# fpusan/moira

Hardware: AMD Instinct MI355X
Metric: reads/sec filtered (300 bp synthetic) (higher is better)
Workload: dtype f64; 1 GPU; BASELINE configs[1]: 10000000 synthetic single-end 300 bp reads, poisson_binomial filter, alpha 0.005, uncert 0.01, resident in HBM (uint8 10000000 x 320, seed 2); reads_per_gpu=10000000, read_length=300, row_stride=320, parallelism=host-side split, 1 rank(s), no data-path collective, world_size=1, mode=bit-exact (no FMA)

## Files before the change

### moira_amd/csrc/mpb_context.cpp

```cpp

#include "mpb_ctx.h"

#include <cstring>
#include <new>


hipError_t Buf::alloc(int64_t bytes)
{
    const hipError_t e = kind == BUF_DEVICE ? hipMalloc(&p, (size_t)bytes)
                                            : hipHostMalloc(&p, (size_t)bytes, kind == BUF_MAPPED ? hipHostMallocMapped : hipHostMallocDefault);
    if (e != hipSuccess) p = nullptr;
    cap = p ? bytes : 0;
    return e;
}

void Buf::release()
{
    if (p) (void)(kind == BUF_DEVICE ? hipFree(p) : hipHostFree(p));
    p = nullptr;
    cap = 0;
}

int Buf::grow(mpb_ctx *c, int64_t bytes, int64_t alloc_bytes)
{
    if (bytes <= cap) return MPB_OK;
    HIPCHK(hipStreamSynchronize(c->stream));
    serve_quiesce(c);
    void *old = p;
    p = nullptr;
    cap = 0;
    if (old) HIPCHK(kind == BUF_DEVICE ? hipFree(old) : hipHostFree(old));
    HIPCHK(alloc(alloc_bytes > bytes ? alloc_bytes : bytes));
    return MPB_OK;
}

int copy_sync(mpb_ctx *c, void *dst, const void *src, size_t bytes, hipMemcpyKind kind)
{
    const hipError_t e_copy = hipMemcpyAsync(dst, src, bytes, kind, c->stream);
    const hipError_t e_sync = hipStreamSynchronize(c->stream);
    HIPCHK_KEPT("hipMemcpyAsync", e_copy);
    HIPCHK_KEPT("hipStreamSynchronize", e_sync);
    return MPB_OK;
}


int mpb_device_count(void)
{
    int n = 0;
    if (hipGetDeviceCount(&n) != hipSuccess) return 0;
    return n;
}

int mpb_create(int device_id, mpb_ctx **out)
{
    if (!out) return fail(MPB_E_INVALID, "mpb_create: out is NULL");
    *out = nullptr;
    int n = mpb_device_count();
    if (n <= 0) return fail(MPB_E_NODEVICE, "no HIP device visible (this library has no CPU path)");
    if (device_id < 0 || device_id >= n)
        return fail(MPB_E_NODEVICE, "device %d out of range (0..%d)", device_id, n - 1);
    HIPCHK(hipSetDevice(device_id));
    mpb_ctx *c = new (std::nothrow) mpb_ctx();
    if (!c) return fail(MPB_E_NOMEM, "host allocation failed");
    c->device = device_id;
    hipError_t e = hipStreamCreateWithFlags(&c->stream, hipStreamNonBlocking);
    if (e == hipSuccess) e = hipStreamCreateWithFlags(&c->copy_stream, hipStreamNonBlocking);
    if (e == hipSuccess) e = hipStreamCreateWithFlags(&c->out_stream, hipStreamNonBlocking);
    for (int k = 0; k < MPB_HOST_SLOTS && e == hipSuccess; k++) {
        e = hipEventCreateWithFlags(&c->slot[k].h2d_done, hipEventDisableTiming);
        if (e == hipSuccess) e = hipEventCreateWithFlags(&c->slot[k].k_done, hipEventDisableTiming);
        if (e == hipSuccess) e = hipEventCreateWithFlags(&c->slot[k].d2h_done, hipEventDisableTiming);
    }
    c->copy_threads = staging_threads();
    auto tables = [c](Carver &k) { k.take(c->d_lut, 256); k.take(c->d_lut_odds, 256); k.take(c->d_lut_private, 256); };
    Carver size;
    tables(size);
    if (e == hipSuccess) e = c->luts.alloc(size.bytes());
    if (e == hipSuccess) {
        Carver place(c->luts.p);
        tables(place);
        MpbPair both[2][256], (&h)[256] = both[0];
        build_lut(both[0], both[1]);
        c->narrow_ok = true;
        for (int qq = 1; qq < 255; qq++) {
            volatile double d = 1.0 - h[qq].y;
            if (memcmp((const void *)&d, &h[qq].x, sizeof(double)) != 0) c->narrow_ok = false;
        }
        e = hipMemcpyAsync(c->d_lut, both, sizeof(both), hipMemcpyHostToDevice, c->stream);
        const hipError_t e_sync = hipStreamSynchronize(c->stream);
        if (e == hipSuccess) e = e_sync;
    }
    if (e == hipSuccess) e = c->pin_mem.alloc(sizeof(PinWords));
    c->pin = (PinWords *)c->pin_mem.p;
    if (e == hipSuccess) {
        hipDeviceProp_t prop;
        e = hipGetDeviceProperties(&prop, device_id);
        if (e == hipSuccess) c->n_cu = prop.multiProcessorCount;
    }
    if (e != hipSuccess) {
        int rc = fail(MPB_E_HIP, "context setup failed: %s", hipGetErrorString(e));
        mpb_destroy(c);
        return rc;
    }
    *out = c;
    return MPB_OK;
}

int mpb_destroy(mpb_ctx *c)
{
    if (!c) return MPB_OK;
    (void)hipSetDevice(c->device);
    serve_free(c);
    if (c->stream) (void)hipStreamSynchronize(c->stream);
    if (c->copy_stream) (void)hipStreamSynchronize(c->copy_stream);
    if (c->out_stream) (void)hipStreamSynchronize(c->out_stream);
    for (auto &sl : c->slot) {
        if (sl.h2d_done) (void)hipEventDestroy(sl.h2d_done);
        if (sl.k_done) (void)hipEventDestroy(sl.k_done);
        if (sl.d2h_done) (void)hipEventDestroy(sl.d2h_done);
    }
    for (auto &s : c->spans) { (void)hipEventDestroy(s.a); (void)hipEventDestroy(s.b); }
    for (auto ev : c->event_pool) (void)hipEventDestroy(ev);
    if (c->stream) (void)hipStreamDestroy(c->stream);
    if (c->copy_stream) (void)hipStreamDestroy(c->copy_stream);
    if (c->out_stream) (void)hipStreamDestroy(c->out_stream);
    delete c;
    return MPB_OK;
}

int mpb_device_lut(mpb_ctx *c, double *a_out, double *b_out)
{
    CTXCHK(c);
    if (!a_out || !b_out) return fail(MPB_E_INVALID, "mpb_device_lut: NULL output");
    double2 h[256];
    int rc = copy_sync(c, h, c->d_lut, sizeof(h), hipMemcpyDeviceToHost);
    if (rc) return rc;
    for (int q = 0; q < 256; q++) { a_out[q] = h[q].x; b_out[q] = h[q].y; }
    return MPB_OK;
}

int mpb_stream(mpb_ctx *c, void **stream_out)
{
    CTXCHK(c);
    if (!stream_out) return fail(MPB_E_INVALID, "stream_out is NULL");
    *stream_out = (void *)c->stream;
    return MPB_OK;
}

int mpb_synchronize(mpb_ctx *c)
{
    CTXCHK(c);
    HIPCHK(hipStreamSynchronize(c->stream));
    return MPB_OK;
}

int mpb_malloc(mpb_ctx *c, int64_t bytes, void **dptr_out)
{
    CTXCHK(c);
    if (!dptr_out || bytes < 0) return fail(MPB_E_INVALID, "mpb_malloc: bad arguments");
    *dptr_out = nullptr;
    HIPCHK(hipMalloc(dptr_out, bytes > 0 ? (size_t)bytes : 16));
    return MPB_OK;
}

int mpb_free(mpb_ctx *c, void *dptr)
{
    CTXCHK(c);
    HIPCHK(hipStreamSynchronize(c->stream));
    serve_quiesce(c);
    if (dptr) HIPCHK(hipFree(dptr));
    return MPB_OK;
}

int mpb_memcpy_h2d(mpb_ctx *c, void *dst, const void *src, int64_t bytes)
{
    CTXCHK(c);
    if (bytes < 0 || (bytes > 0 && (!dst || !src))) return fail(MPB_E_INVALID, "mpb_memcpy_h2d: bad arguments");
    if (bytes == 0) return MPB_OK;
    return copy_sync(c, dst, src, (size_t)bytes, hipMemcpyHostToDevice);
}

int mpb_memcpy_d2h(mpb_ctx *c, void *dst, const void *src, int64_t bytes)
{
    CTXCHK(c);
    if (bytes < 0 || (bytes > 0 && (!dst || !src))) return fail(MPB_E_INVALID, "mpb_memcpy_d2h: bad arguments");
    if (bytes == 0) return MPB_OK;
    return copy_sync(c, dst, src, (size_t)bytes, hipMemcpyDeviceToHost);
}

int mpb_memset(mpb_ctx *c, void *dst, int value, int64_t bytes)
{
    CTXCHK(c);
    if (bytes < 0 || (bytes > 0 && !dst)) return fail(MPB_E_INVALID, "mpb_memset: bad arguments");
    if (bytes == 0) return MPB_OK;
    HIPCHK(hipMemsetAsync(dst, value, (size_t)bytes, c->stream));
    return MPB_OK;
}

int mpb_host_alloc(mpb_ctx *c, int64_t bytes, void **hptr_out)
{
    CTXCHK(c);
    if (!hptr_out || bytes < 0) return fail(MPB_E_INVALID, "mpb_host_alloc: bad arguments");
    *hptr_out = nullptr;
    HIPCHK(hipHostMalloc(hptr_out, bytes > 0 ? (size_t)bytes : 16, hipHostMallocDefault));
    return MPB_OK;
}

int mpb_host_free(mpb_ctx *c, void *hptr)
{
    CTXCHK(c);
    drain_pipeline(c);
    serve_quiesce(c);
    if (hptr) HIPCHK(hipHostFree(hptr));
    return MPB_OK;
}


int ensure_workspace(mpb_ctx *c, int64_t n)
{
    if (!c->ws_small.p) {
        int rc = c->ws_small.grow(c, sizeof(MpbSmallBlock));
        if (rc) return rc;
        HIPCHK(hipMemsetAsync(c->ws_small.p, 0, sizeof(MpbSmallBlock), c->stream));
        MpbSmallBlock *b = (MpbSmallBlock *)c->ws_small.p;
        c->ws.tables = &b->tables;
        c->ws.tables2 = &b->tables2;
        c->ws.ovf_count = &b->ovf_count;
        c->ws.bad_len = &b->bad_len;
        c->ws.pass_count = &b->pass_count;
        c->ws.ovf_total = &b->ovf_total;
        c->ws.wide_count = &b->wide_count;
        c->ws.alg_cells = &b->alg_cells;
        c->ws.nar_count = &b->nar_count;
        c->ws.nar_sample = b->nar_sample;
        c->ws.pt_count = &b->pt_count;
        c->ws.lut = c->d_lut;
    }
    if (n <= c->ws_cap) return MPB_OK;
    c->ws_cap = 0;
    const int64_t cap = n + n / 8 + 1024;
    const int64_t nb = (cap + MPB_PRE_READS - 1) / MPB_PRE_READS;
    MpbWorkspace &w = c->ws;
    int rc = carve(c, c->ws_block, [&w, cap, nb](Carver &k) {
        k.take(w.cls, cap);
        k.take(w.perm, cap + (int64_t)MPB_NCLS * 64);
        k.take(w.perm_ns, cap + (int64_t)MPB_NCLS * 64);
        k.take(w.blockhist, nb * MPB_SKEYS);
        k.take(w.ovf_list, cap);
    });
    if (rc) return rc;
    c->ws_cap = cap;
    return MPB_OK;
}

int ensure_wide_workspace(mpb_ctx *c, int64_t n)
{
    if (n <= c->ws_wide_cap) return MPB_OK;
    c->ws_wide_cap = 0;
    const int64_t cap = n + n / 8 + 1024;
    MpbWorkspace &w = c->ws;
    int rc = carve(c, c->ws_wide, [&w, cap](Carver &k) { k.take(w.wide_list, cap); k.take(w.wide_rows, cap); });
    if (rc) return rc;
    c->ws_wide_cap = cap;
    return MPB_OK;
}

int ensure_narrow_workspace(mpb_ctx *c, int64_t n, bool ragged)
{
    const int64_t cap = n + n / 8 + 1024;
    MpbWorkspace &w = c->ws;
    int rc;
    if (n > c->ws_nar_cap) {
        c->ws_nar_cap = 0;
        rc = carve(c, c->ws_nar, [&w, cap](Carver &k) {
            k.take(w.nar_seg, cap + 64);
            k.take(w.nar_list, cap + 64);
            k.take(w.nar_wave_count, MPB_NAR_MAX_WAVES + 1);
        });
        if (rc) return rc;
        c->ws_nar_cap = cap;
    }
    if (ragged && n > c->ws_rg_cap) {
        c->ws_rg_cap = 0;
        rc = carve(c, c->ws_rg, [&w, cap](Carver &k) {
            k.take(w.rg_ord, cap + 64);
            k.take(w.rg_gpre, cap / 64 + 2);
            k.take(w.rg_wsum, cap / 4096 + 2);
            k.take(w.rg_wpre, cap / 4096 + 2);
            k.take(w.rg_gstart, MPB_NAR_MAX_WAVES + 1);
        });
        if (rc) return rc;
        c->ws_rg_cap = cap;
        if (!c->rg_per_cu[0]) mpb_narrow_rg_blocks_per_cu(c->rg_per_cu);
    }
    return MPB_OK;
}

int PrivateTable::install(const double2 *h)
{
    int rc = ensure_workspace(c, 1);
    if (rc) return rc;
    if ((rc = copy_sync(c, c->d_lut_private, h, 256 * sizeof(double2), hipMemcpyHostToDevice))) return rc;
    c->ws.lut = c->d_lut_private;
    on = true;
    return MPB_OK;
}


static hipEvent_t get_event(mpb_ctx *c)
{
    if (!c->event_pool.empty()) { hipEvent_t e = c->event_pool.back(); c->event_pool.pop_back(); return e; }
    hipEvent_t e = nullptr;
    (void)hipEventCreate(&e);
    return e;
}


void Span::start()
{
    a = get_event(c); b = get_event(c);
    (void)hipEventRecord(a, c->stream);
}

static int resolve_spans(mpb_ctx *c)
{
    if (c->spans.empty()) return MPB_OK;
    HIPCHK(hipStreamSynchronize(c->stream));
    for (auto &s : c->spans) {
        float ms = 0.f;
        if (hipEventElapsedTime(&ms, s.a, s.b) == hipSuccess) { c->acc_ms[s.kid] += ms; c->acc_n[s.kid] += 1; }
        c->event_pool.push_back(s.a);
        c->event_pool.push_back(s.b);
    }
    c->spans.clear();
    return MPB_OK;
}

int mpb_timing_enable(mpb_ctx *c, int on) { CTXCHK(c); c->timing = on != 0; return MPB_OK; }

int mpb_timing_reset(mpb_ctx *c)
{
    CTXCHK(c);
    int rc = resolve_spans(c);
    if (rc) return rc;
    for (int k = 0; k < MPB_K_COUNT; k++) { c->acc_ms[k] = 0; c->acc_n[k] = 0; }
    return MPB_OK;
}

int mpb_kernel_time(mpb_ctx *c, int kid, double *total_ms, int64_t *launches)
{
    CTXCHK(c);
    if (kid < 0 || kid >= MPB_K_COUNT) return fail(MPB_E_INVALID, "kernel id %d out of range", kid);
    int rc = resolve_spans(c);
    if (rc) return rc;
    if (total_ms) *total_ms = c->acc_ms[kid];
    if (launches) *launches = c->acc_n[kid];
    return MPB_OK;
}
```

### moira_amd/csrc/mpb_ctx.h

```cpp
#ifndef MPB_CTX_H
#define MPB_CTX_H

#include "../../include/moira_pb.h"
#include "mpb_internal.h"
#include "mpb_host_internal.h"
#include "mpb_hostonly.h"

#include <vector>

static_assert(sizeof(MpbPair) == sizeof(double2) && offsetof(MpbPair, y) == sizeof(double), "MpbPair is double2's layout");

static inline int hip_fail(const char *what, hipError_t e)
{
    return fail(e == hipErrorOutOfMemory ? MPB_E_NOMEM : MPB_E_HIP, "%s failed: %s", what, hipGetErrorString(e));
}
#define HIPCHK(expr)                                        \
    do {                                                    \
        hipError_t e_ = (expr);                             \
        if (e_ != hipSuccess) return hip_fail(#expr, e_);   \
    } while (0)
#define HIPCHK_KEPT(what, e)                                \
    do {                                                    \
        if ((e) != hipSuccess) return hip_fail(what, e);    \
    } while (0)

#define CTXCHK(c)                                                     \
    do {                                                              \
        if (!(c)) return fail(MPB_E_INVALID, "%s: ctx is NULL", __func__); \
        HIPCHK(hipSetDevice((c)->device));                            \
    } while (0)

enum BufKind { BUF_DEVICE, BUF_PINNED, BUF_MAPPED };
struct Buf {
    BufKind kind;
    void *p = nullptr;
    int64_t cap = 0;
    explicit Buf(BufKind k = BUF_DEVICE) : kind(k) {}
    Buf(const Buf &) = delete;
    Buf &operator=(const Buf &) = delete;
    ~Buf() { release(); }
    hipError_t alloc(int64_t bytes);
    int grow(mpb_ctx *c, int64_t bytes, int64_t alloc_bytes = 0);
    void release();
};

struct Carver {
    char *base;
    int64_t off = 0;
    explicit Carver(void *b = nullptr) : base((char *)b) {}
    template <typename T> void take(T *&ptr, int64_t count)
    {
        ptr = base ? (T *)(base + off) : nullptr;
        off += align_up(count * (int64_t)sizeof(T), 256);
    }
    int64_t bytes() const { return off; }
};
template <typename Layout>
static int carve(mpb_ctx *c, Buf &b, Layout &&layout, int headroom = 1)
{
    Carver size;
    layout(size);
    int rc = b.grow(c, size.bytes(), size.bytes() * headroom);
    if (rc) return rc;
    Carver place(b.p);
    layout(place);
    return MPB_OK;
}

struct MpbSmallBlock {
    alignas(256) MpbTables tables;
    alignas(256) MpbTables tables2;
    alignas(64) int32_t ovf_count;
    alignas(64) int32_t bad_len;
    alignas(64) unsigned long long pass_count;
    alignas(64) long long ovf_total;
    alignas(64) int32_t wide_count;
    alignas(64) unsigned long long alg_cells;
    alignas(64) int32_t nar_count;
    alignas(64) int32_t nar_sample[MPB_NAR_BUCKETS + 2];
    alignas(64) int32_t pt_count;
};

struct PinWords {
    int32_t nar_count;
    int32_t n_overflow;
    unsigned long long n_pass;
    int32_t bad_len;
    int32_t bad255;
    int32_t sample[MPB_NAR_BUCKETS + 2];
    int32_t pt_handed;
    unsigned long long pt_kept;
    long long ovf_total;
    int64_t text_status[2];
    uint32_t fq_head[4];
    int64_t fq_status[4];
    uint32_t fq_head2[4];
    int64_t fq_status2[4];
    int64_t pair_status[4];
    uint32_t pair_head[MPB_PAIR_HEAD_WORDS];
    int64_t fmt_words[2];
};

struct TimedSpan { int kid; hipEvent_t a, b; };

struct ChunkArrays {
    uint8_t *q; int32_t *len; double *ee; int32_t *ns; uint8_t *pass;
    void in(Carver &k, int64_t m, int64_t row_stride) { k.take(q, m * row_stride); k.take(len, m); }
    void out(Carver &k, int64_t m) { k.take(ee, m); k.take(ns, m); k.take(pass, m); }
};

#define MPB_HOST_SLOTS 4
struct HostSlot {
    Buf dev{BUF_DEVICE}, pin_in{BUF_PINNED}, pin_out{BUF_PINNED};
    ChunkArrays d{}, hin{}, hout{};
    hipEvent_t h2d_done = nullptr, k_done = nullptr, d2h_done = nullptr;
    int64_t off = -1, m = 0;
};

struct mpb_ctx {
    int device = -1;
    hipStream_t stream = nullptr;
    hipStream_t copy_stream = nullptr;
    hipStream_t out_stream = nullptr;
    HostSlot slot[MPB_HOST_SLOTS];
    int copy_threads = 1;
    Buf luts{BUF_DEVICE};
    double2 *d_lut = nullptr;
    double2 *d_lut_odds = nullptr;
    double2 *d_lut_private = nullptr;
    MpbWorkspace ws{};
    Buf ws_small{BUF_DEVICE};
    Buf ws_block{BUF_DEVICE};
    int64_t ws_cap = 0;
    struct Classified {
        bool valid = false; const uint8_t *q = nullptr; int64_t n = 0, stride = 0; const int32_t *len = nullptr;
        int32_t fixed_len = 0; mpb_filter_params params{}; double *ee = nullptr; int32_t *ns = nullptr; uint8_t *pass = nullptr;
    } classified;
    Buf ws_wide{BUF_DEVICE};
    int64_t ws_wide_cap = 0;
    bool timing = false;
    std::vector<TimedSpan> spans;
    std::vector<hipEvent_t> event_pool;
    double acc_ms[MPB_K_COUNT] = {0};
    int64_t acc_n[MPB_K_COUNT] = {0};
    Buf stage{BUF_DEVICE};
    Buf pin_host{BUF_MAPPED};
    uint32_t small_token = 0;
    int n_cu = 0;
    bool narrow_ok = false;
    Buf ws_nar{BUF_DEVICE};
    int64_t ws_nar_cap = 0;
    Buf ws_rg{BUF_DEVICE}; int64_t ws_rg_cap = 0;
    Buf pt_rec{BUF_DEVICE};
    int rg_per_cu[MPB_NRG_FORMS] = {0};
    Buf text_stage{BUF_DEVICE};
    Buf contig_stage{BUF_DEVICE};
    Buf contig_tabs{BUF_DEVICE};
    bool contig_tabs_ready = false;
    Buf bgzf_stage{BUF_DEVICE};
    Buf inflate_stage{BUF_DEVICE};
    Buf fastq_stage{BUF_DEVICE};
    Buf fastq_index{BUF_DEVICE};
    Buf format_stage{BUF_DEVICE};
    Buf format_out{BUF_DEVICE};
    struct ResidentText {
        int64_t gen = 0, last = 0;
        const uint8_t *text = nullptr; int64_t text_bytes = 0; const int64_t *idx = nullptr; int64_t n = 0;
    } resident;
    Buf pin_mem{BUF_PINNED};
    PinWords *pin = nullptr;
    struct NarrowChoice {
        bool valid = false; int64_t n = 0, stride = 0; int32_t fixed_len = 0; double alpha = 0; uint32_t flags = 0;
        int rows0 = 0; int split = 0; int calls = 0;
        double expect_back = 0;
    } nar_choice;
    mpb_path_info last_path{};
    bool classes_whole = true;
    struct CtxServe {
        bool tried = false, ok = false, running = false;
        hipStream_t stream = nullptr;
        Buf pin{BUF_MAPPED}, dev{BUF_DEVICE};
        MpbServeBox box{};
        uint32_t generation = 0, tok = 0;
        double cached_alpha = -1.0;
        MpbDevParams cached_prm;
    } serve;
};

struct Span {
    mpb_ctx *c; int kid; hipEvent_t a = nullptr, b = nullptr;
    Span(mpb_ctx *c_, int kid_) : c(c_), kid(kid_) { if (c->timing) start(); }
    void start();
    ~Span()
    {
        if (c->timing) { (void)hipEventRecord(b, c->stream); c->spans.push_back({kid, a, b}); }
    }
};

#include "mpb_queue.h"

struct PrivateTable {
    mpb_ctx *c;
    bool on = false;
    explicit PrivateTable(mpb_ctx *ctx) : c(ctx) {}
    int install(const double2 *h);
    ~PrivateTable() { if (on) c->ws.lut = c->d_lut; }
};

int copy_sync(mpb_ctx *c, void *dst, const void *src, size_t bytes, hipMemcpyKind kind);
int ensure_workspace(mpb_ctx *c, int64_t n);
int ensure_wide_workspace(mpb_ctx *c, int64_t n);
int ensure_narrow_workspace(mpb_ctx *c, int64_t n, bool ragged);
MpbDevParams make_dev_params(const mpb_filter_params *p, int32_t fixed_len, int32_t max_len);
void drain_pipeline(mpb_ctx *c);
int filter_host_pipeline(mpb_ctx *c, const uint8_t *q, int64_t n, int64_t row_stride, const int32_t *len, int32_t fixed_len,
                         const mpb_filter_params *params, double *ee, int32_t *ns, uint8_t *pass, mpb_filter_counts *counts,
                         int poisson);
struct TextStage {
    uint8_t *text; mpb_text_row *rows; int64_t *status; uint8_t *q; int32_t *len; uint8_t *flags;
    double *ee; int32_t *ns; uint8_t *pass;
    void layout(Carver &k, int64_t text_bytes, int64_t n, int64_t piece_rows, int64_t stride)
    {
        k.take(text, align_up(text_bytes > 0 ? text_bytes : 1, 16));
        k.take(rows, n);
        layout_results(k, n, piece_rows, stride);
    }
    void layout_results(Carver &k, int64_t n, int64_t piece_rows, int64_t stride)
    {
        k.take(status, 2);
        k.take(q, piece_rows * stride);
        k.take(len, n); k.take(flags, n);
        k.take(ee, n); k.take(ns, n); k.take(pass, n);
    }
};
int64_t text_piece_rows(int64_t n, int64_t stride);
int filter_text_pieces(StreamQueue &q, const uint8_t *d_text, int64_t text_bytes, const mpb_text_row *d_rows, int64_t n, int64_t stride,
                       int64_t piece_rows, int32_t fastq_offset, int32_t lower_n_is_base, const mpb_filter_params *params,
                       int32_t poisson, const TextStage &st, int64_t *n_pass, int64_t *n_overflow, int64_t *bad_record);
struct TextResults {
    double *ee; int32_t *ns; uint8_t *pass; int32_t *len; uint8_t *flags;
    std::vector<int32_t> len_tmp;
    int32_t *len_host() const { return len ? len : len_tmp.empty() ? nullptr : const_cast<int32_t *>(len_tmp.data()); }
};
static inline bool text_host_tail(const mpb_filter_params *params, int32_t poisson)
{
    return poisson && !(params && (params->flags & MPB_FLAG_POISSON_DEVICE_TAIL));
}
int text_results_queue(StreamQueue &q, const TextStage &st, int64_t n, bool host_tail, TextResults &r);
int text_results_tail(int64_t n, const mpb_filter_params *params, bool host_tail, const TextResults &r, int64_t *n_pass);
int text_results_out(StreamQueue &q, const TextStage &st, int64_t n, const mpb_filter_params *params, int32_t poisson, TextResults &r,
                     int64_t *n_pass);

struct FastqStage {
    uint8_t *text; uint32_t *info, *prefix, *head; int64_t *status;
    void layout(Carver &k, int64_t text_bytes, int64_t n_tiles)
    {
        k.take(text, align_up(text_bytes > 0 ? text_bytes : 1, 16));
        k.take(info, n_tiles > 0 ? n_tiles : 1);
        k.take(prefix, n_tiles > 0 ? n_tiles : 1);
        k.take(head, 4);
        k.take(status, 4);
    }
};

struct FastqIndex {
    uint32_t *start; int64_t *idx; uint8_t *kinds; mpb_text_row *desc;
    void layout(Carver &k, int64_t n_start, int64_t rows)
    {
        k.take(start, n_start);
        k.take(idx, rows * MPB_IDX_COLS);
        k.take(kinds, rows);
        k.take(desc, rows);
    }
};

struct Indexed {
    FastqStage st{};
    FastqIndex ix{};
    int64_t n = 0, rows = 0, longest = 0;
};
void fastq_index_queue_head(StreamQueue &q, Indexed &out, int64_t text_bytes, int32_t final, uint32_t *pin_head = nullptr);
int fastq_index_finish(StreamQueue &q, int64_t text_bytes, int64_t max_records, int32_t max_len, int64_t idx_cap_rows, int64_t *n_needed,
                       Indexed &out, int32_t *why);
void queue_index_out(StreamQueue &q, const Indexed &in, int64_t *idx_out, uint32_t *consumed32, uint8_t *kind8);
struct FastqFilterAsk {
    int32_t fastq_offset, lower_n_is_base; const mpb_filter_params *params; int32_t poisson;
    mpb_filter_counts *counts; int64_t *bad_record;
};
int filter_indexed(StreamQueue &q, const Indexed &in, int64_t text_bytes, uint8_t *text_out, int64_t *idx_out, int64_t *n,
                   int64_t *consumed, int32_t *bad_kind, const FastqFilterAsk &ask, TextResults &r);
void resident_keep(mpb_ctx *c, const Indexed &in, int64_t text_bytes);
void resident_drop(mpb_ctx *c);
struct BgzfStage {
    uint8_t *text; uint32_t *tok; uint8_t *slots; uint32_t *size, *mstat, *crc; int64_t *off; uint8_t *out;
    void layout(Carver &k, int64_t members)
    {
        k.take(text, align_up(members * (int64_t)MPB_BGZF_DATA, 16));
        k.take(tok, members * (int64_t)MPB_BGZF_DATA);
        k.take(slots, members * (int64_t)MPB_BGZF_SLOT);
        k.take(size, members); k.take(mstat, members * 4); k.take(crc, members);
        k.take(off, members + 1);
        k.take(out, members * ((int64_t)MPB_BGZF_DATA + 31));
    }
};
struct BgzfHost {
    std::vector<uint32_t> crc, mstat;
    std::vector<int64_t> off;
    int reserve(int64_t per_piece);
};
int64_t bgzf_piece_members(int64_t members);
int bgzf_compress_piece(StreamQueue &q, const BgzfStage &st, int64_t tb, int64_t nm, const uint8_t *host_text,
                        const mpb_crc_range *d_ranges, uint32_t *d_bad, BgzfHost &h, uint8_t *out, int64_t out_room, int64_t *got_out,
                        mpb_bgzf_stats *stats);
void serve_quiesce(mpb_ctx *c);
void serve_free(mpb_ctx *c);

#endif
```

### moira_amd/csrc/mpb_internal.h

```cpp
#ifndef MPB_INTERNAL_H
#define MPB_INTERNAL_H

#include <hip/hip_runtime.h>
#include "mpb_shared.h"

#define MPB_TILE_MAX_ROWS 1024
#define MPB_WIDE_WAVES 16
#define MPB_MAX_ROWS (MPB_TILE_MAX_ROWS * MPB_WIDE_WAVES)
#define MPB_MAX_STRIDE 65536
#define MPB_SMALL_MAX_STRIDE 16384

struct MpbClass { int cap, G, R; };

#define MPB_NCLS 32
#define MPB_CLASSES(X)                                                                       \
    X(0, 2, 1) X(1, 3, 1) X(2, 4, 1) X(3, 5, 1) X(4, 6, 1) X(5, 7, 1) X(6, 8, 1) X(7, 9, 1)  \
    X(8, 10, 1) X(9, 12, 1) X(10, 14, 1) X(11, 16, 1)                                        \
    X(12, 10, 2) X(13, 12, 2) X(14, 14, 2) X(15, 16, 2)                                      \
    X(16, 10, 4) X(17, 12, 4) X(18, 14, 4) X(19, 16, 4)                                      \
    X(20, 9, 8) X(21, 10, 8) X(22, 11, 8) X(23, 12, 8) X(24, 14, 8) X(25, 16, 8)             \
    X(26, 10, 16) X(27, 12, 16) X(28, 16, 16)                                                \
    X(29, 12, 32) X(30, 16, 32) X(31, 16, 64)

#define MPB_THIN_CLASSES(X)                                                                  \
    X(0, 1, 2) X(1, 1, 4) X(2, 1, 8) X(3, 1, 16) X(4, 1, 32) X(5, 1, 64) X(6, 2, 64)         \
    X(7, 4, 64) X(8, 8, 64) X(9, 16, 64)

#define MPB_CLASS_ENTRY(ID, RR, GG) {(RR) * (GG), GG, RR},
#define MPB_CLASS_TABLE { MPB_CLASSES(MPB_CLASS_ENTRY) }

#define MPB_PRE_ROUNDS 4
#define MPB_PRE_READS (256 * MPB_PRE_ROUNDS)
#define MPB_CLS_SETTLED 0x7f
#define MPB_CLS_WIDE 0x7e

#define MPB_LEN_SHIFT 6
#define MPB_LEN_BINS (1024 >> MPB_LEN_SHIFT)
#define MPB_SKEYS (MPB_NCLS * MPB_LEN_BINS)

struct MpbTables {
    int32_t count[MPB_NCLS];
    int32_t perm_base[MPB_NCLS + 1];
    int32_t tile_start[MPB_NCLS + 1];
    int32_t total_tiles;
    int32_t kcount[MPB_SKEYS];
    int32_t key_base[MPB_SKEYS];
};

#define MPB_DP_CHUNK 8

struct MpbDevParams {
    double thr;
    double uncert;
    double maxerrors;
    float  z;
    float  zq;
    float  clow;
    int32_t ambig_mode;
    uint32_t flags;
    int32_t fixed_len;
    int32_t max_len;
    int32_t len_shift;
};

struct MpbWorkspace {
    uint8_t  *cls;
    int32_t  *perm;
    uint16_t *perm_ns;
    int32_t  *blockhist;
    MpbTables *tables;
    MpbTables *tables2;
    int32_t  *ovf_list;
    int32_t  *ovf_count;
    int32_t  *bad_len;
    long long *ovf_total;
    int32_t  *wide_list;
    int32_t  *wide_rows;
    int32_t  *wide_count;
    unsigned long long *pass_count;
    unsigned long long *alg_cells;
    const double2 *lut;
    int32_t  *nar_count;
    int32_t  *nar_seg;
    int32_t  *nar_list;
    int32_t  *nar_wave_count;
    int32_t  *nar_sample;
    int2     *rg_ord;
    int32_t  *rg_gpre;
    unsigned long long *rg_wsum, *rg_wpre;
    int32_t  *rg_gstart;
    int32_t  *pt_count;
};

#define MPB_NAR_MAX_WAVES 8192
#define MPB_NAR_AUTO_MIN_READS (1 << 18)

#define MPB_LUT_BYTES   (256 * 16)
#define MPB_LAMBDA_MAX_STRIDE (1 << 24)

void mpb_launch_prepass(const uint8_t *q, int64_t n, int64_t stride, const int32_t *len,
                        const MpbDevParams &prm, const MpbWorkspace &ws, int32_t *ns_out,
                        double *ee_out, uint8_t *pass_out, hipStream_t s, const int32_t *list = nullptr);
void mpb_launch_decode_classify(const uint8_t *seq, const uint8_t *qual, int32_t offset, uint8_t *out, int32_t *err,
                                int64_t n, int64_t stride, const int32_t *len, const MpbDevParams &prm,
                                const MpbWorkspace &ws, int32_t *ns_out, double *ee_out, uint8_t *pass_out, hipStream_t s);
void mpb_launch_encode(const uint8_t *q, int64_t n, int64_t stride, int32_t offset, uint8_t *seq, uint8_t *qual, hipStream_t s);
struct MpbSmallHost {
    uint8_t *stage;
    int32_t *ns_dev;
    uint32_t *done;
    uint32_t token;
};
void mpb_launch_small(const uint8_t *q, int64_t n, int64_t stride, const int32_t *len, const MpbDevParams &prm,
                      const MpbWorkspace &ws, int32_t *ns, double *ee, uint8_t *pass, hipStream_t s,
                      const MpbSmallHost *host = nullptr);
#define MPB_SERVE_STRIDE 2048
struct alignas(64) MpbServePrm { MpbDevParams p; };
struct MpbServeBox {
    const uint8_t *q;
    int64_t stride;
    const MpbServePrm *prm;
    const unsigned long long *door;
    uint32_t *done;
    double *ee; int32_t *ns; uint8_t *pass;
    int64_t q_step, prm_step, door_step, done_step, ee_step, ns_step, pass_step;
    const uint32_t *stop;
    uint32_t *exited;
    uint8_t *stage;
    int32_t *ns_dev; uint8_t *cls; int32_t *ident;
    uint32_t *gone;
    int32_t n_ent;
};
void mpb_launch_serve(const MpbServeBox &box, const double2 *lut, uint32_t generation, uint32_t lifetime_ms, hipStream_t s);
void mpb_launch_scan(int64_t n, const int32_t *len, const MpbWorkspace &ws, hipStream_t s);
void mpb_launch_scatter(int64_t n, const int32_t *len, const int32_t *ns, const MpbDevParams &prm, const MpbWorkspace &ws,
                        hipStream_t s, const int32_t *list = nullptr);
void mpb_launch_dp(const uint8_t *q, int64_t n, int64_t stride, const int32_t *len,
                   const MpbDevParams &prm, const MpbWorkspace &ws, const int32_t *ns,
                   double *ee, uint8_t *pass, hipStream_t s, const double2 *lut_odds = nullptr);
void mpb_launch_overflow(const uint8_t *q, int64_t n, int64_t stride, const int32_t *len,
                         const MpbDevParams &prm, const MpbWorkspace &ws, const int32_t *ns,
                         double *ee, uint8_t *pass, hipStream_t s);
void mpb_launch_wide(const uint8_t *q, int64_t stride, const int32_t *len, const MpbDevParams &prm,
                     const MpbWorkspace &ws, const int32_t *ns, double *ee, uint8_t *pass, hipStream_t s);
void mpb_launch_lambda(const uint8_t *q, int64_t n, int64_t stride, const int32_t *len, int32_t fixed_len,
                       const double2 *lut_ap, double *lambda, int32_t *ns, int32_t *bad, hipStream_t s);
#define MPB_PT_LAMBDA_MAX 64.0
#define MPB_PT_WINDOW 0x1p-17
struct MpbPoissonRec { double lambda; int32_t idx, ns, len, pad_; };
struct MpbPoissonFix { double ee; int32_t idx, pass; };
void mpb_launch_poisson_tail(const double *lambda, const int32_t *ns, const int32_t *len, int64_t n, const MpbDevParams &prm,
                             double *ee, uint8_t *pass, int32_t *handed, MpbPoissonRec *rec, int32_t rec_cap,
                             unsigned long long *n_pass, hipStream_t s);
void mpb_launch_poisson_patch(const MpbPoissonFix *fix, int32_t m, double *ee, uint8_t *pass, hipStream_t s);
void mpb_launch_decode(const uint8_t *seq, const uint8_t *qual, int64_t n, int64_t stride, const int32_t *len,
                       int32_t fixed_len, int32_t offset, uint8_t *out, int32_t *err, hipStream_t s);
void mpb_launch_count(const uint8_t *pass, int64_t n, const MpbWorkspace &ws, hipStream_t s);
void mpb_launch_pack_text(const uint8_t *text, int64_t text_bytes, const mpb_text_row *rows, int64_t n, int64_t k0, int32_t offset,
                          bool lower_n_is_base, int64_t stride, uint8_t *out, int32_t *len_out, uint8_t *flags_out,
                          int64_t *status, hipStream_t s);
#define MPB_RG_MAX_STRIDE 4096
#define MPB_NRG_FORMS 8
#define MPB_NRG_EXACT_FORMS 5
#define MPB_NAR_GRID_CAP_MAX 2048
void mpb_launch_narrow(int rows0, int split_chunks, const uint8_t *q, int64_t n, int64_t stride, int32_t fixed_len, const int32_t *len,
                       const MpbDevParams &prm, const MpbWorkspace &ws, double *ee, int32_t *ns, uint8_t *pass, int n_cu,
                       const int *rg_per_cu, int grid_cap, int *waves, hipStream_t s, const double2 *lut_odds = nullptr);
void mpb_narrow_rg_blocks_per_cu(int per_cu[MPB_NRG_FORMS]);
void mpb_launch_sample(const uint8_t *q, int64_t n, int64_t stride, int32_t fixed_len, const int32_t *len, const MpbDevParams &prm,
                       const MpbWorkspace &ws, int n_sample, hipStream_t s);
struct MpbContigArgs;
void mpb_launch_contigs(const MpbContigArgs &a, hipStream_t s);
void mpb_launch_contig_rows(const int64_t *out_idx, const uint8_t *done, int64_t n, int64_t rec_cap, int32_t max_len, int64_t stride,
                            mpb_text_row *rows, hipStream_t s);
#define MPB_BGZF_SLOT 65536
void mpb_launch_bgzf_deflate(const uint8_t *text, int64_t text_bytes, int64_t n_members, uint32_t *tok, uint8_t *slots,
                             uint32_t *size, uint32_t *mstat, hipStream_t s);
void mpb_launch_bgzf_scan(const uint32_t *size, int64_t n_members, int64_t *off, hipStream_t s);
void mpb_launch_bgzf_frame(const uint8_t *slots, const uint32_t *size, const int64_t *off, const uint32_t *crc, int64_t text_bytes,
                           int64_t n_members, int64_t out_cap, uint8_t *out, hipStream_t s);
#define MPB_INFLATE_MSTAT 8
void mpb_launch_bgzf_inflate(const uint8_t *in, int64_t in_bytes, const mpb_bgzf_member_row *rows, int64_t n_members, uint8_t *text,
                             int64_t text_bytes, uint32_t *mstat, hipStream_t s);
#define MPB_FQ_TILE 16384
void mpb_launch_fq_lines(const uint8_t *text, int64_t text_bytes, int64_t n_tiles, uint32_t *info, hipStream_t s);
void mpb_launch_fq_scan(const uint8_t *text, int64_t text_bytes, bool final_text, const uint32_t *info, int64_t n_tiles,
                        uint32_t *prefix, uint32_t *head, hipStream_t s);
void mpb_launch_fq_starts(const uint8_t *text, int64_t text_bytes, int64_t n_tiles, const uint32_t *prefix, const uint32_t *head,
                          uint32_t *start, int64_t n_start, hipStream_t s);
void mpb_launch_fq_rows(const uint8_t *text, int64_t text_bytes, const uint32_t *start, int64_t n_start, int64_t n, int32_t max_len,
                        int64_t *idx, uint8_t *kinds, mpb_text_row *desc, int64_t *status, hipStream_t s);
#define MPB_CRC_RANGE_MAX 65536
struct mpb_crc_range { int64_t off; int32_t len, pad; };
void mpb_launch_bgzf_crc32(const uint8_t *text, int64_t text_bytes, const mpb_crc_range *ranges, int64_t n, uint32_t *crc,
                           uint32_t *bad, hipStream_t s);
#define MPB_PAIR_HEAD_WORDS 32
struct MpbLdsClasses;
void mpb_launch_pair_rows(const int64_t *fidx, const int64_t *ridx, int64_t m, const uint8_t *ftext, int64_t fbytes, const uint8_t *rtext,
                          int64_t rbytes, int maxabs, bool take, const MpbLdsClasses &classes, mpb_pair_row *rows, int8_t *cls,
                          int64_t *status, hipStream_t s);
void mpb_launch_pair_count(const mpb_pair_row *rows, const int8_t *cls, int64_t n, uint32_t *table, uint32_t *prefix, uint32_t *head,
                           int64_t *status, hipStream_t s);
void mpb_launch_pair_lists(const int8_t *cls, int64_t n, const uint32_t *prefix, const uint32_t *head, int32_t *list, hipStream_t s);
struct FmParams;
void mpb_launch_fmt_count(const uint8_t *text, const int64_t *idx, const int64_t *sel, const int64_t *relabel_index,
                          const int32_t *label_id, int64_t nsel, const FmParams &p, int64_t *size, int64_t *prefix, int64_t *head,
                          int64_t *status, hipStream_t s);
void mpb_launch_fmt_write(const uint8_t *text, const uint8_t *blob, const int64_t *idx, const int64_t *sel,
                          const int64_t *relabel_index, const int32_t *label_id, int64_t k0, int64_t k1, const FmParams &p,
                          const int64_t *prefix, const int64_t *status, int64_t win_lo, int64_t win_hi, uint8_t *out, hipStream_t s);
void mpb_launch_synth(uint8_t *q, int64_t n, int64_t stride, int32_t fixed_len, int32_t min_len,
                      int32_t max_len, int32_t *len, uint64_t seed, int64_t first_read,
                      hipStream_t s, int32_t profile = 0);

#endif
```

### moira_amd/csrc/mpb_kernels.hip

```cpp

#include "mpb_internal.h"
#include <cstdlib>
#include <cstdio>
#include "../../include/mpb_synth.h"

#pragma clang fp contract(off)

__shared__ double2 mpb_s_lut[256];
__shared__ unsigned long long mpb_s_cells;

namespace {

__constant__ MpbClass c_classes[MPB_NCLS] = MPB_CLASS_TABLE;

struct ClassOfRows {
    uint8_t t[MPB_TILE_MAX_ROWS + 1];
    constexpr ClassOfRows() : t{}
    {
        constexpr MpbClass cl[MPB_NCLS] = MPB_CLASS_TABLE;
        for (int rows = 0; rows < MPB_TILE_MAX_ROWS + 1; rows++) {
            int c = 0;
            for (int k = 0; k < MPB_NCLS - 1; k++) c += (rows > cl[k].cap) ? 1 : 0;
            t[rows] = (uint8_t)c;
        }
    }
};
__constant__ ClassOfRows c_class_of_rows{};

__device__ __forceinline__ int lane_id() { return threadIdx.x & 63; }

template <typename T>
__device__ __forceinline__ T gload(const T *p)
{
    return *(const __attribute__((address_space(1))) T *)(p);
}
typedef uint32_t u32x4 __attribute__((ext_vector_type(4)));
__device__ __forceinline__ uint4 gload16(const uint8_t *p)
{
    const u32x4 x = *(const __attribute__((address_space(1))) u32x4 *)(p);
    return make_uint4(x.x, x.y, x.z, x.w);
}
template <typename T>
__device__ __forceinline__ void gstore(T *p, T v)
{
    *(__attribute__((address_space(1))) T *)(p) = v;
}

__device__ __forceinline__ void wave_lds_fence()
{
    __builtin_amdgcn_fence(__ATOMIC_RELEASE, "wavefront");
    __builtin_amdgcn_s_waitcnt(0xc07f);
    __builtin_amdgcn_wave_barrier();
    __builtin_amdgcn_fence(__ATOMIC_ACQUIRE, "wavefront");
}

__device__ __forceinline__ int clamp_len(int li, int max_len) { return min(max(li, 0), max_len); }

__device__ __forceinline__ bool settled_by_chernoff(const MpbDevParams &prm, float mu, int li)
{
    if (!(prm.flags & MPB_FLAG_DECISION_ONLY)) return false;
    const float t = mu * (1.0f - 1e-4f) - prm.clow * sqrtf(mu) - 0.02f;
    return mu > 1.0f && (double)floorf(t) > mpb_limit(prm, li);
}

typedef float f32x2 __attribute__((ext_vector_type(2)));

__device__ __forceinline__ uint32_t mask_dword(uint32_t w, int nvalid_bytes)
{
    if (nvalid_bytes >= 4) return w;
    if (nvalid_bytes <= 0) return 0u;
    return w & ((1u << (8 * nvalid_bytes)) - 1u);
}

__device__ __forceinline__ uint32_t fill_dword(uint32_t w, int nvalid_bytes)
{
    if (nvalid_bytes >= 4) return w;
    if (nvalid_bytes <= 0) return 0xFEFEFEFEu;
    const uint32_t m = (1u << (8 * nvalid_bytes)) - 1u;
    return (w & m) | (0xFEFEFEFEu & ~m);
}

#define MPB_PRE_NB 5
#define MPB_MARK_UPPER 128.0f
#define MPB_MARK_LOWER 65536.0f

__device__ __forceinline__ void pre_chunk(const float2 *tab, const uint4 x, f32x2 &a01, float &s3)
{
    const uint32_t ww[4] = {x.x, x.y, x.z, x.w};
#pragma unroll
    for (int d = 0; d < 4; d++)
#pragma unroll
        for (int t = 0; t < 4; t++) {
            const float2 e = tab[(ww[d] >> (8 * t)) & 0xffu];
            a01 += (f32x2){e.x, e.y};
            s3 = __builtin_fmaf(e.x, e.y, s3);
        }
}

__device__ __forceinline__ uint32_t decode4_bytes(uint32_t sw, uint32_t qw, int nv, int offset, int &bad)
{
    uint32_t ow = 0;
#pragma unroll
    for (int t = 0; t < 4; t++) {
        const uint32_t b = (sw >> (8 * t)) & 0xffu;
        int qv = (int)((qw >> (8 * t)) & 0xffu) - offset;
        uint32_t o = 0;
        if (t < nv) {
            if (qv < 0) { bad++; qv = 1; }
            if (qv > 254) { bad++; qv = 254; }
            if (qv == 0) qv = 1;
            o = b == 'N' ? 0u : b == 'n' ? 255u : (uint32_t)qv;
        }
        ow |= o << (8 * t);
    }
    return ow;
}

__device__ __forceinline__ uint32_t zero_bytes(uint32_t x)
{
    return ~(((x & 0x7f7f7f7fu) + 0x7f7f7f7fu) | x) & 0x80808080u;
}

__device__ __forceinline__ uint32_t decode4(uint32_t sw, uint32_t qw, int nv, int offset, uint32_t off4, int &bad)
{
    const uint32_t H = 0x80808080u;
    const uint32_t d = ((qw | H) - (off4 & ~H)) ^ ((qw ^ ~off4) & H);
    uint32_t lt = ((~qw & off4) | (~(qw ^ off4) & d)) & H;
    uint32_t keep = 0xffffffffu;
    if (nv < 4) keep = nv <= 0 ? 0u : ((1u << (8 * nv)) - 1u);
    lt &= keep;
    if (lt) return decode4_bytes(sw, qw, nv, offset, bad);
    uint32_t q = d + (zero_bytes(d) >> 7);
    const uint32_t amb = zero_bytes((sw | 0x20202020u) ^ 0x6e6e6e6eu);
    const uint32_t amb_full = (amb << 1) - (amb >> 7);
    const uint32_t lower_full = ((sw >> 5) & 0x01010101u) * 255u;
    q = (amb_full & lower_full) | (~amb_full & q);
    return q & keep;
}

__device__ __forceinline__ uint4 decode16(const uint4 sq, const uint4 ql, int pos0, int li, int offset, int &bad)
{
    const int nv = li - pos0;
    if (offset < 1)
        return make_uint4(decode4_bytes(sq.x, ql.x, nv, offset, bad), decode4_bytes(sq.y, ql.y, nv - 4, offset, bad),
                          decode4_bytes(sq.z, ql.z, nv - 8, offset, bad), decode4_bytes(sq.w, ql.w, nv - 12, offset, bad));
    const uint32_t off4 = (uint32_t)(offset & 0xff) * 0x01010101u;
    if (offset > 255) {
        return make_uint4(decode4_bytes(sq.x, ql.x, nv, offset, bad), decode4_bytes(sq.y, ql.y, nv - 4, offset, bad),
                          decode4_bytes(sq.z, ql.z, nv - 8, offset, bad), decode4_bytes(sq.w, ql.w, nv - 12, offset, bad));
    }
    return make_uint4(decode4(sq.x, ql.x, nv, offset, off4, bad), decode4(sq.y, ql.y, nv - 4, offset, off4, bad),
                      decode4(sq.z, ql.z, nv - 8, offset, off4, bad), decode4(sq.w, ql.w, nv - 12, offset, off4, bad));
}

__device__ __forceinline__ uint32_t lower_as_q254(uint32_t w)
{
    return w ^ (zero_bytes(~w) >> 7);
}

__device__ __forceinline__ void pre_dword_again(const float2 *tab, uint32_t w, f32x2 &a01, float &s3)
{
    w = lower_as_q254(w);
#pragma unroll 1
    for (int t = 0; t < 4; t++) {
        const float2 e = tab[(w >> (8 * t)) & 0xffu];
        a01 += (f32x2){e.x, e.y};
        s3 = __builtin_fmaf(e.x, e.y, s3);
    }
}

struct PreDecode {
    const uint8_t *seq;
    const uint8_t *qual;
    uint8_t *out;
    int32_t offset;
    int32_t *err;
};

struct PreOut {
    uint8_t *cls; int32_t *ns; double *ee; uint8_t *pass;
    int32_t *bad_len, *wide_list, *wide_rows, *wide_count;
};

__device__ __forceinline__ void class_read(int64_t i, float mu, float var, float k3, uint32_t ambi, int li, bool bad, bool ragged,
                                           const MpbDevParams &prm, const PreOut &o, int *s_hist, int nb)
{
    const int nzero = (int)(ambi & 0xffffu), n255 = (int)(ambi >> 16);
    const float v = fmaxf(var, 1e-12f);
    const float x = mu + prm.z * sqrtf(v) + (k3 / v) * prm.zq;
    int rows = (int)floorf(fminf(x, 1e9f) + 0.5f) + 1;
    if (prm.flags & MPB_FLAG_TEST_UNDERPREDICT) rows = rows / 2;
    const int scored = li - nzero - n255;
    rows = min(rows, scored + 1);
    rows = max(rows, 1);
    o.ns[i] = bad ? 0 : nzero + n255;
    const int c = c_class_of_rows.t[min(rows, MPB_TILE_MAX_ROWS)];
    const bool settled = !bad && settled_by_chernoff(prm, mu, li);
    const bool empty = !bad && scored <= 0 && !(1.0 > prm.thr);
    if (bad) {
        atomicAdd(o.bad_len, 1);
        o.cls[i] = (uint8_t)MPB_CLS_SETTLED;
        o.ee[i] = __builtin_nan("");
        o.pass[i] = 0;
    } else if (empty) {
        double e = mpb_add_ns(prm, 0.0, nzero + n255);
        const bool keep = mpb_round_and_keep(prm, e, nzero > 0, li);
        o.cls[i] = (uint8_t)(MPB_CLS_SETTLED | (nzero > 0 ? 0x80 : 0));
        o.ee[i] = e;
        o.pass[i] = (uint8_t)(keep ? 1 : 0);
    } else if (settled) {
        o.cls[i] = (uint8_t)(MPB_CLS_SETTLED | (nzero > 0 ? 0x80 : 0));
        o.ee[i] = __builtin_inf();
        o.pass[i] = 0;
    } else if (rows > MPB_TILE_MAX_ROWS) {
        const int pos = atomicAdd(o.wide_count, 1);
        o.wide_list[pos] = (int32_t)i;
        o.wide_rows[pos] = rows;
        o.cls[i] = (uint8_t)(MPB_CLS_WIDE | (nzero > 0 ? 0x80 : 0));
    } else {
        o.cls[i] = (uint8_t)(c | (nzero > 0 ? 0x80 : 0));
        atomicAdd(&s_hist[c * nb + (ragged ? min(MPB_LEN_BINS - 1, li >> prm.len_shift) : 0)], 1);
    }
}

template <bool RAGGED, bool LONG, bool LISTED>
__global__ __launch_bounds__(256) void k_prepass(const uint8_t *__restrict__ q, int64_t n,
                                                 int64_t stride, const int32_t *__restrict__ len_arg,
                                                 MpbDevParams prm, PreOut o, int32_t *__restrict__ blockhist,
                                                 const int32_t *__restrict__ list)
{
    __shared__ float2 s_tab[256];
    __shared__ float4 s_row[4][64];
    __shared__ int s_hist[RAGGED ? MPB_SKEYS : MPB_NCLS];
    const int32_t *__restrict__ len = RAGGED ? len_arg : nullptr;
    constexpr int nb = RAGGED ? MPB_LEN_BINS : 1;
    const int tid = threadIdx.x, w = tid >> 6, lane = tid & 63;
    {
        const bool amb = tid == 0 || tid == 255;
        float p = __builtin_amdgcn_exp2f(-0.33219281f * (float)tid);
        p = amb ? 0.0f : p;
        s_tab[tid] = make_float2(p, tid == 0 ? MPB_MARK_UPPER : tid == 255 ? MPB_MARK_LOWER : p * (1.0f - p));
    }
    for (int k = tid; k < MPB_NCLS * nb; k += 256) s_hist[k] = 0;
    __syncthreads();

    const int r16 = lane & 15, cl = lane >> 4;
    for (int round = 0; round < MPB_PRE_ROUNDS; round++) {
    const int64_t wave_row0 = (int64_t)blockIdx.x * MPB_PRE_READS + round * 256 + w * 64;
    if (wave_row0 >= n) break;

    for (int rb = 0; rb < 64; rb += 16) {
        const bool live = wave_row0 + rb + r16 < n;
        const int64_t i = LISTED ? (live ? (int64_t)list[wave_row0 + rb + r16] : 0) : wave_row0 + rb + r16;
        const int li = live ? (len ? clamp_len(len[i], prm.max_len) : prm.fixed_len) : 0;
        int ncol = (li + 15) >> 4;
        int nfull = live ? (li >> 4) : (1 << 20);
        if (len || wave_row0 + 64 > n) {
#pragma unroll
            for (int off = 8; off >= 1; off >>= 1) {
                ncol = max(ncol, __shfl_xor(ncol, off));
                nfull = min(nfull, __shfl_xor(nfull, off));
            }
        }
        ncol = __builtin_amdgcn_readfirstlane(ncol);
        nfull = __builtin_amdgcn_readfirstlane(nfull);
        const uint8_t *src = q + (live ? i : (int64_t)0) * stride + cl * 16;
        float mu = 0.f, var = 0.f, k3 = 0.f;
        uint32_t ambi = 0;
        auto panel = [&](const int pb, const int pend) {
        f32x2 a01 = {0.f, 0.f};
        float s3 = 0.f;
        for (int cb = pb; cb < pend; cb += 4 * MPB_PRE_NB) {
            uint4 xs[MPB_PRE_NB];
#pragma unroll
            for (int b = 0; b < MPB_PRE_NB; b++) {
                const int c0 = cb + 4 * b;
                xs[b] = make_uint4(0, 0, 0, 0);
                if (c0 < pend && li > (c0 + cl) * 16)
                    xs[b] = *reinterpret_cast<const uint4 *>(src + c0 * 16);
            }
#pragma unroll
            for (int b = 0; b < MPB_PRE_NB; b++) {
                const int c0 = cb + 4 * b;
                if (c0 >= pend) break;
                uint4 y = xs[b];
                if (c0 + 4 > nfull) {
                    const int nv = li - (c0 + cl) * 16;
                    y.x = fill_dword(y.x, nv); y.y = fill_dword(y.y, nv - 4);
                    y.z = fill_dword(y.z, nv - 8); y.w = fill_dword(y.w, nv - 12);
                }
                pre_chunk(s_tab, y, a01, s3);
            }
        }
        const float n255 = floorf(a01.y * (1.0f / MPB_MARK_LOWER));
        if (n255 > 0.0f) {
            a01 = (f32x2){0.f, 0.f};
            s3 = 0.f;
#pragma unroll 1
            for (int c0 = pb; c0 < pend; c0 += 4) {
                const int nv = li - (c0 + cl) * 16;
                if (nv <= 0) break;
#pragma unroll 1
                for (int d = 0; d < 4; d++)
                    pre_dword_again(s_tab, fill_dword(*reinterpret_cast<const uint32_t *>(src + c0 * 16 + d * 4), nv - 4 * d), a01, s3);
            }
        }
        const float rem = a01.y;
        const float nzero = floorf(rem * (1.0f / MPB_MARK_UPPER));
        const float pvar = rem - MPB_MARK_UPPER * nzero;
        mu += a01.x;
        var += pvar;
        k3 += pvar - 2.0f * s3;
        ambi += (uint32_t)nzero + ((uint32_t)n255 << 16);
        };
        if (LONG) { for (int pb = 0; pb < ncol; pb += 12 * MPB_PRE_NB) panel(pb, min(ncol, pb + 12 * MPB_PRE_NB)); }
        else panel(0, ncol);
#pragma unroll
        for (int off = 16; off <= 32; off <<= 1) {
            mu += __shfl_xor(mu, off);
            var += __shfl_xor(var, off);
            k3 += __shfl_xor(k3, off);
            ambi += __shfl_xor(ambi, off);
        }
        const float amb = __uint_as_float(ambi);
        if (cl == 0) s_row[w][rb + r16] = make_float4(mu, var, k3, amb);
    }
    wave_lds_fence();
    {
        const int64_t k = wave_row0 + lane;
        if (k < n) {
            const int64_t i = LISTED ? (int64_t)list[k] : k;
            const float4 e = s_row[w][lane];
            const int li = len ? clamp_len(len[i], prm.max_len) : prm.fixed_len;
            class_read(i, e.x, e.y, e.z, __float_as_uint(e.w), li, RAGGED && li != len[i], RAGGED, prm, o, s_hist, nb);
        }
    }
    wave_lds_fence();
    }
    __syncthreads();
    for (int k = tid; k < MPB_NCLS * nb; k += 256) blockhist[(int64_t)k * gridDim.x + blockIdx.x] = s_hist[k];
}

#define MPB_LIN_K 5
#define MPB_LIN_CHUNKS (256 * MPB_LIN_K)

template <bool RAGGED, bool DECODE>
__global__ __launch_bounds__(256) void k_classify_linear(const uint8_t *__restrict__ q, int64_t n, int64_t stride,
                                                         const int32_t *__restrict__ len_arg, MpbDevParams prm, PreOut o,
                                                         int32_t *__restrict__ blockhist, PreDecode dec, uint32_t cpr_magic)
{
    __shared__ float2 s_tab[256];
    __shared__ float4 s_part[MPB_LIN_CHUNKS];
    __shared__ int s_len[MPB_PRE_READS];
    __shared__ int s_hist[RAGGED ? MPB_SKEYS : MPB_NCLS];
    const int32_t *__restrict__ len = RAGGED ? len_arg : nullptr;
    constexpr int nb = RAGGED ? MPB_LEN_BINS : 1;
    const int tid = threadIdx.x;
    {
        const bool amb = tid == 0 || tid == 255;
        float p = __builtin_amdgcn_exp2f(-0.33219281f * (float)tid);
        p = amb ? 0.0f : p;
        s_tab[tid] = make_float2(p, tid == 0 ? MPB_MARK_UPPER : tid == 255 ? MPB_MARK_LOWER : p * (1.0f - p));
    }
    for (int k = tid; k < MPB_NCLS * nb; k += 256) s_hist[k] = 0;
    const int cpr = (int)(stride >> 4);
    const int tile_rows = max(1, min(MPB_PRE_READS, MPB_LIN_CHUNKS / cpr));
    const int64_t first = (int64_t)blockIdx.x * MPB_PRE_READS;
    const int64_t last = min(n, first + MPB_PRE_READS);
    int lpr = 1;
    while (lpr < 64 && lpr * 2 * tile_rows <= 256) lpr *= 2;
    int badq = 0;
    for (int64_t row0 = first; row0 < last; row0 += tile_rows) {
        const int nr = (int)min((int64_t)tile_rows, last - row0);
        const int nchunks = nr * cpr;
        __syncthreads();
        for (int t = tid; t < nr; t += 256) s_len[t] = len ? clamp_len(len[row0 + t], prm.max_len) : prm.fixed_len;
        __syncthreads();
        const int64_t base = row0 * stride;
        uint4 xs[MPB_LIN_K], ys[MPB_LIN_K];
        int nvs[MPB_LIN_K];
#pragma unroll
        for (int k = 0; k < MPB_LIN_K; k++) {
            const int c = tid + k * 256;
            xs[k] = ys[k] = make_uint4(0, 0, 0, 0);
            nvs[k] = -1;
            if (c < nchunks) {
                const int r = cpr_magic ? (int)__umulhi((uint32_t)c, cpr_magic) : c;
                const int col = c - r * cpr;
                const int nv = s_len[r] - col * 16;
                nvs[k] = max(nv, 0);
                if (nv > 0) {
                    if (DECODE) {
                        xs[k] = *reinterpret_cast<const uint4 *>(dec.seq + base + (int64_t)c * 16);
                        ys[k] = *reinterpret_cast<const uint4 *>(dec.qual + base + (int64_t)c * 16);
                    } else {
                        xs[k] = *reinterpret_cast<const uint4 *>(q + base + (int64_t)c * 16);
                    }
                }
            }
        }
        __builtin_amdgcn_sched_barrier(0);
#pragma unroll
        for (int k = 0; k < MPB_LIN_K; k++) {
            const int c = tid + k * 256;
            const int nv = nvs[k];
            if (nv < 0) continue;
            uint4 y = xs[k];
            if (DECODE) {
                if (nv > 0) y = decode16(xs[k], ys[k], 0, nv, dec.offset, badq);
                *reinterpret_cast<uint4 *>(dec.out + base + (int64_t)c * 16) = y;
            }
            float4 part = make_float4(0.f, 0.f, 0.f, __int_as_float(0));
            if (nv > 0) {
                if (nv < 16) {
                    y.x = fill_dword(y.x, nv); y.y = fill_dword(y.y, nv - 4);
                    y.z = fill_dword(y.z, nv - 8); y.w = fill_dword(y.w, nv - 12);
                }
                f32x2 a01 = {0.f, 0.f};
                float s3 = 0.f;
                pre_chunk(s_tab, y, a01, s3);
                const float n255 = floorf(a01.y * (1.0f / MPB_MARK_LOWER));
                if (n255 > 0.0f) {
                    a01 = (f32x2){0.f, 0.f};
                    s3 = 0.f;
                    pre_dword_again(s_tab, y.x, a01, s3); pre_dword_again(s_tab, y.y, a01, s3);
                    pre_dword_again(s_tab, y.z, a01, s3); pre_dword_again(s_tab, y.w, a01, s3);
                }
                const float rem = a01.y;
                const float nzero = floorf(rem * (1.0f / MPB_MARK_UPPER));
                const float pvar = rem - MPB_MARK_UPPER * nzero;
                part = make_float4(a01.x, pvar, pvar - 2.0f * s3, __uint_as_float((uint32_t)nzero + ((uint32_t)n255 << 16)));
            }
            s_part[c] = part;
        }
        __syncthreads();
        const int sub = tid & (lpr - 1);
        for (int r = tid / lpr; r < nr; r += 256 / lpr) {
            float mu = 0.f, var = 0.f, k3 = 0.f;
            uint32_t ambi = 0;
            for (int j = sub; j < cpr; j += lpr) {
                const float4 e = s_part[r * cpr + j];
                mu += e.x; var += e.y; k3 += e.z; ambi += __float_as_uint(e.w);
            }
            for (int off = 1; off < lpr; off <<= 1) {
                mu += __shfl_xor(mu, off); var += __shfl_xor(var, off);
                k3 += __shfl_xor(k3, off); ambi += __shfl_xor(ambi, off);
            }
            if (sub == 0) {
                const int64_t i = row0 + r;
                const int li = s_len[r];
                class_read(i, mu, var, k3, ambi, li, RAGGED && li != len[i], RAGGED, prm, o, s_hist, nb);
            }
        }
    }
    if (DECODE && badq && dec.err) atomicAdd(dec.err, badq);
    __syncthreads();
    for (int k = tid; k < MPB_NCLS * nb; k += 256) blockhist[(int64_t)k * gridDim.x + blockIdx.x] = s_hist[k];
}

__global__ __launch_bounds__(256) void k_scan(int32_t *__restrict__ blockhist, int nblocks,
                                              MpbTables *__restrict__ tb)
{
    __shared__ int s_part[256];
    const int c = blockIdx.x, tid = threadIdx.x;
    const int seg = (nblocks + 255) / 256;
    const int b0 = tid * seg, b1 = min(nblocks, b0 + seg);
    int sum = 0;
    int32_t *bh = blockhist + (int64_t)c * nblocks;
    for (int b = b0; b < b1; b++) sum += bh[b];
    s_part[tid] = sum;
    __syncthreads();
    for (int off = 1; off < 256; off <<= 1) {
        int v = (tid >= off) ? s_part[tid - off] : 0;
        __syncthreads();
        s_part[tid] += v;
        __syncthreads();
    }
    int run = s_part[tid] - sum;
    for (int b = b0; b < b1; b++) {
        const int h = bh[b];
        bh[b] = run;
        run += h;
    }
    if (tid == 255) tb->kcount[c] = s_part[255];
}

__global__ __launch_bounds__(512) void k_tables(MpbTables *__restrict__ tb, int nb, int32_t *__restrict__ ovf_count,
                                                unsigned long long *__restrict__ pass_count)
{
    __shared__ int s_k[MPB_SKEYS], s_cnt[MPB_NCLS], s_base[MPB_NCLS + 1], s_tile[MPB_NCLS + 1];
    const int tid = threadIdx.x;
    for (int k = tid; k < MPB_NCLS * nb; k += 512) s_k[k] = tb->kcount[k];
    __syncthreads();
    if (tid < MPB_NCLS) {
        int cnt = 0;
        for (int b = 0; b < nb; b++) cnt += s_k[tid * nb + b];
        s_cnt[tid] = cnt;
    }
    __syncthreads();
    if (tid == 0) {
        int base = 0;
        for (int c = 0; c < MPB_NCLS; c++) { s_base[c] = base; base += (s_cnt[c] + 63) & ~63; }
        s_base[MPB_NCLS] = base;
        int t = 0;
        for (int c = MPB_NCLS - 1; c >= 0; c--) {
            const int rpt = 64 / c_classes[c].G;
            s_tile[c] = t;
            t += (s_cnt[c] + rpt - 1) / rpt;
        }
        s_tile[MPB_NCLS] = t;
    }
    __syncthreads();
    if (tid < MPB_NCLS) {
        const int c = tid;
        tb->perm_base[c] = s_base[c];
        tb->count[c] = s_cnt[c];
        tb->tile_start[c] = s_tile[c];
        int run = s_base[c];
        for (int b = 0; b < nb; b++) {
            tb->key_base[c * nb + b] = run;
            run += s_k[c * nb + b];
        }
    }
    if (tid == 0) {
        tb->perm_base[MPB_NCLS] = s_base[MPB_NCLS];
        tb->tile_start[MPB_NCLS] = s_tile[MPB_NCLS];
        tb->total_tiles = s_tile[MPB_NCLS];
        *ovf_count = 0;
        *pass_count = 0ull;
    }
}

__global__ void k_tables_overflow(MpbTables *__restrict__ tb, const int32_t *__restrict__ ovf_count,
                                  int wc, long long *__restrict__ ovf_total)
{
    if (threadIdx.x != 0 || blockIdx.x != 0) return;
    const int cnt = *ovf_count;
    *ovf_total += cnt;
    const int rpt = 64 / c_classes[wc].G;
    for (int c = 0; c <= MPB_NCLS; c++) {
        if (c < MPB_NCLS) tb->count[c] = (c == wc) ? cnt : 0;
        tb->perm_base[c] = 0;
        tb->tile_start[c] = 0;
    }
    tb->total_tiles = (cnt + rpt - 1) / rpt;
}

template <bool RAGGED>
__global__ __launch_bounds__(256) void k_scatter(const uint8_t *__restrict__ cls, int64_t n,
                                                 const int32_t *__restrict__ len_arg, int max_len, int len_shift,
                                                 const int32_t *__restrict__ blockhist,
                                                 const MpbTables *__restrict__ tb,
                                                 const int32_t *__restrict__ ns,
                                                 int32_t *__restrict__ perm, uint16_t *__restrict__ perm_ns,
                                                 const int32_t *__restrict__ list)
{
    constexpr int nb = RAGGED ? MPB_LEN_BINS : 1;
    constexpr int nkeys = MPB_NCLS * nb;
    __shared__ int s_wcnt[4][nkeys];
    __shared__ int s_base[nkeys];
    const int32_t *__restrict__ len = RAGGED ? len_arg : nullptr;
    const int tid = threadIdx.x, w = tid >> 6, lane = tid & 63;
    for (int k = tid; k < nkeys; k += 256) s_base[k] = tb->key_base[k] + blockhist[(int64_t)k * gridDim.x + blockIdx.x];
    int kk_r[MPB_PRE_ROUNDS], ns_r[MPB_PRE_ROUNDS], c_r[MPB_PRE_ROUNDS], len_r[MPB_PRE_ROUNDS], id_r[MPB_PRE_ROUNDS];
#pragma unroll
    for (int round = 0; round < MPB_PRE_ROUNDS; round++) {
        const int64_t k = (int64_t)blockIdx.x * MPB_PRE_READS + round * 256 + tid;
        const int64_t i = (list && k < n) ? (int64_t)list[k] : k;
        id_r[round] = (int)i;
        c_r[round] = k < n ? (int)cls[i] : 0xff;
        ns_r[round] = k < n ? ns[i] : 0;
        len_r[round] = (len && k < n) ? len[i] : 0;
    }
#pragma unroll
    for (int round = 0; round < MPB_PRE_ROUNDS; round++) {
        int c = c_r[round] == 0xff ? -1 : (c_r[round] & 0x7f);
        if (c >= MPB_NCLS) c = -1;
        kk_r[round] = c < 0 ? -1 : c * nb + (len ? min(MPB_LEN_BINS - 1, clamp_len(len_r[round], max_len) >> len_shift) : 0);
    }
#pragma unroll
    for (int round = 0; round < MPB_PRE_ROUNDS; round++) {
        for (int k = tid; k < 4 * nkeys; k += 256) (&s_wcnt[0][0])[k] = 0;
        __syncthreads();
        const int kk = kk_r[round];
        int rank = 0;
        unsigned long long remaining = __ballot(kk >= 0);
        while (remaining) {
            const int leader = __ffsll((long long)remaining) - 1;
            const int cc = __shfl(kk, leader);
            const unsigned long long m = __ballot(kk == cc);
            if (kk == cc) rank = __popcll(m & ((1ull << lane) - 1ull));
            if (lane == leader) s_wcnt[w][cc] = __popcll(m);
            remaining &= ~m;
        }
        __syncthreads();
        if (kk >= 0) {
            int off = s_base[kk];
            for (int ww = 0; ww < w; ww++) off += s_wcnt[ww][kk];
            perm[off + rank] = (int32_t)id_r[round];
            perm_ns[off + rank] = (uint16_t)ns_r[round];
        }
        __syncthreads();
        for (int k = tid; k < nkeys; k += 256)
            s_base[k] += s_wcnt[0][k] + s_wcnt[1][k] + s_wcnt[2][k] + s_wcnt[3][k];
        __syncthreads();
    }
}

__device__ __forceinline__ double dpp_prev_row(double x, int keep)
{
    const long long k64 = ((long long)keep << 32) | (unsigned int)keep;
    const long long y = __builtin_amdgcn_update_dpp(0ll, __double_as_longlong(x), 0x138, 0xf, 0xf, true) & k64;
    return __longlong_as_double(y);
}

template <bool FMA>
__device__ __forceinline__ double cell(double a, double v, double b, double w)
{
    if (FMA) return __builtin_fma(a, v, b * w);
    const double x = a * v;
    const double y = b * w;
    return x + y;
}

enum { MPB_AR_EXACT = 0, MPB_AR_FMA = 1, MPB_AR_ODDS = 2 };

template <int R, int G, int AR>
__device__ __forceinline__ void dp_step(double (&v)[R], double &p0, const double2 ab, const int keep)
{
    double cin = 0.0;
    if (G > 1) cin = dpp_prev_row(v[R - 1], keep);
    if (AR == MPB_AR_ODDS) {
#pragma unroll
        for (int r = R - 1; r >= 1; r--) v[r] = __builtin_fma(ab.y, v[r - 1], v[r]);
        if (G > 1) v[0] = __builtin_fma(ab.y, cin, v[0]);
        p0 *= ab.x;
        return;
    }
#pragma unroll
    for (int r = R - 1; r >= 1; r--) v[r] = cell<AR == MPB_AR_FMA>(ab.x, v[r], ab.y, v[r - 1]);
    if (G > 1) v[0] = cell<AR == MPB_AR_FMA>(ab.x, v[0], ab.y, cin);
    else v[0] = ab.x * v[0];
}

template <int R, int G, int AR>
__device__ __forceinline__ void dp_dword(double (&v)[R], double &p0, uint32_t w, int keep)
{
#pragma unroll
    for (int t = 0; t < 4; t++) dp_step<R, G, AR>(v, p0, mpb_s_lut[(w >> (8 * t)) & 0xffu], keep);
}

template <int R, int G, int AR>
__device__ __forceinline__ void dp_chunk_compact(double (&v)[R], double &p0, const uint4 x, int keep)
{
    uint32_t w0 = x.x, w1 = x.y, w2 = x.z, w3 = x.w;
#pragma unroll 1
    for (int d = 0; d < 2; d++) {
        dp_dword<R, G, AR>(v, p0, w0, keep);
        dp_dword<R, G, AR>(v, p0, w1, keep);
        w0 = w2; w1 = w3;
    }
}

template <int R, int G, int AR>
__device__ __forceinline__ void dp_chunk_tail(double (&v)[R], double &p0, const uint4 x, int keep, int ndw)
{
    uint32_t w0 = x.x, w1 = x.y, w2 = x.z, w3 = x.w;
    int d = 0;
#pragma unroll 1
    for (; d + 2 <= ndw; d += 2) {
        dp_dword<R, G, AR>(v, p0, w0, keep);
        dp_dword<R, G, AR>(v, p0, w1, keep);
        w0 = w2; w1 = w3;
    }
    if (d < ndw) dp_dword<R, G, AR>(v, p0, w0, keep);
}

template <int R, int G, int AR>
__device__ __forceinline__ void dp_chunk(double (&v)[R], double &p0, const uint4 x, int keep)
{
    if (R <= 8) {
        dp_dword<R, G, AR>(v, p0, x.x, keep);
        dp_dword<R, G, AR>(v, p0, x.y, keep);
        dp_dword<R, G, AR>(v, p0, x.z, keep);
        dp_dword<R, G, AR>(v, p0, x.w, keep);
    } else {
        dp_chunk_compact<R, G, AR>(v, p0, x, keep);
    }
}

template <int R>
__device__ __forceinline__ int cdf_cross(const double (&v)[R], double acc, double thr, int j0, double &lo, double &hi)
{
    int js = -1;
#pragma unroll
    for (int r = 0; r < R; r++) {
        const double na = acc + v[r];
        const bool hit = (js < 0) && (na > thr);
        lo = hit ? acc : lo;
        hi = hit ? na : hi;
        js = hit ? j0 + r : js;
        acc = na;
    }
    return js;
}

__device__ __forceinline__ double cross_ee(bool crossed, int js, double thr, double lo, double hi)
{
    if (!crossed) return __builtin_nan("");
    double e = (double)(js - 1) + ((thr - lo) / (hi - lo));
    if (e < 0) e = 0;
    return e;
}

__device__ __forceinline__ double cross_ee_odds(bool crossed, int js, double thr, double p0, double lo, double hi)
{
    if (!crossed) return __builtin_nan("");
    double e = (double)(js - 1) + (__builtin_fma(-lo, p0, thr) / (p0 * (hi - lo)));
    if (e < 0) e = 0;
    return e;
}

__device__ __forceinline__ bool read_result(const MpbDevParams &prm, bool crossed, int js, double lo, double hi, int nsv, bool has_n,
                                            int li, double &e)
{
    e = mpb_add_ns(prm, cross_ee(crossed, js, prm.thr, lo, hi), nsv);
    return mpb_round_and_keep(prm, e, has_n, li);
}

__device__ __forceinline__ bool mode_unsure(const MpbDevParams &prm, double e, int li)
{
    const double tol = 1e-9 * fmax(1.0, fabs(e));
    bool unsure = fabs(e - mpb_limit(prm, li)) <= tol;
    if (prm.flags & MPB_FLAG_ROUND) unsure = unsure || fabs(e - rint(e)) <= tol;
    return unsure;
}

#define MPB_DP_WAVES_PER_EU 4

struct DpArgs {
    const uint8_t *q;
    int64_t stride;
    const int32_t *len;
    const int32_t *ns;
    const uint8_t *cls;
    double *ee;
    uint8_t *pass;
    int32_t *ovf_list;
    int32_t *ovf_count;
    unsigned long long *alg_cells;
    const int32_t *perm;
    const uint16_t *perm_ns;
    MpbDevParams prm;
    int final_pass;
};

__device__ __forceinline__ bool class_has_n(const DpArgs &A, int idx)
{
    return A.prm.ambig_mode == MPB_AMBIG_DISALLOW && (gload(A.cls + idx) & 0x80);
}

#define MPB_DP_AR (FMA ? MPB_AR_FMA : MPB_AR_EXACT)
template <int R, int G, bool FMA>
__device__ __noinline__ void dp_tiles(const DpArgs *__restrict__ Ap, const int32_t *perm_cls,
                                      int count, int first_tile, int n_tiles)
#include "mpb_dp_tiles.inc"
#undef MPB_DP_AR

#define MPB_DP_AR MPB_AR_ODDS
template <int R, int G>
__device__ __noinline__ void dp_tiles_odds(const DpArgs *__restrict__ Ap, const int32_t *perm_cls,
                                           int count, int first_tile, int n_tiles)
#include "mpb_dp_tiles.inc"
#undef MPB_DP_AR


template <int AR>
__device__ __forceinline__ void dp_grid(const DpArgs &args, DpArgs &s_args, const double2 *__restrict__ lut_g,
                                        MpbTables *__restrict__ tb, const int32_t *__restrict__ perm, int chunk_tiles)
{
    mpb_s_lut[threadIdx.x] = lut_g[threadIdx.x];
    if (threadIdx.x == 0) { s_args = args; mpb_s_cells = 0ull; }
    __syncthreads();
    const DpArgs *A = &s_args;
    const int total = tb->total_tiles;
    const int nchunks = (total + chunk_tiles - 1) / chunk_tiles;
    for (int chunk = blockIdx.x * 4 + (threadIdx.x >> 6); chunk < nchunks; chunk += gridDim.x * 4) {
        const int t0 = chunk * chunk_tiles;
        const int t1 = min(total, t0 + chunk_tiles);
        for (int c = MPB_NCLS - 1; c >= 0; c--) {
            const int cnt = tb->count[c];
            const int rpt = 64 / c_classes[c].G;
            const int s = tb->tile_start[c];
            const int e = s + (cnt + rpt - 1) / rpt;
            const int lo = max(t0, s), hi = min(t1, e);
            if (lo >= hi) continue;
            const int32_t *pc = perm + tb->perm_base[c];
            switch (c) {
#define MPB_CASE(ID, RR, GG) case ID:                                                                 \
                if constexpr (AR == MPB_AR_ODDS) dp_tiles_odds<RR, GG>(A, pc, cnt, lo - s, hi - lo);                \
                else dp_tiles<RR, GG, AR == MPB_AR_FMA>(A, pc, cnt, lo - s, hi - lo);                     \
                break;
                MPB_CLASSES(MPB_CASE)
#undef MPB_CASE
            default: break;
            }
        }
    }
    if (args.prm.flags & MPB_FLAG_COUNT_CELLS) {
        __syncthreads();
        if (threadIdx.x == 0 && mpb_s_cells) atomicAdd(args.alg_cells, mpb_s_cells);
    }
}

template <bool FMA, bool OVERFLOW_PASS>
__global__ __launch_bounds__(256, MPB_DP_WAVES_PER_EU) void k_dp(DpArgs args,
                                            const double2 *__restrict__ lut_g,
                                            MpbTables *__restrict__ tb,
                                            const int32_t *__restrict__ perm, int chunk_tiles)
{
    __shared__ DpArgs s_args;
    dp_grid<FMA ? MPB_AR_FMA : MPB_AR_EXACT>(args, s_args, lut_g, tb, perm, chunk_tiles);
}

__global__ __launch_bounds__(256, MPB_DP_WAVES_PER_EU) void k_dp_odds(DpArgs args,
                                            const double2 *__restrict__ lut_g,
                                            MpbTables *__restrict__ tb,
                                            const int32_t *__restrict__ perm, int chunk_tiles)
{
    __shared__ DpArgs s_args;
    dp_grid<MPB_AR_ODDS>(args, s_args, lut_g, tb, perm, chunk_tiles);
}

#define MPB_WIDE_R 16

__device__ __forceinline__ void wide_report(const DpArgs &A, int idx, int li, bool crossed, int js, double lo, double hi)
{
    double e;
    const bool keep_read = read_result(A.prm, crossed, js, lo, hi, gload(A.ns + idx), class_has_n(A, idx), li, e);
    gstore(A.ee + idx, e);
    gstore(A.pass + idx, (uint8_t)(keep_read ? 1 : 0));
}

template <bool FINAL, int W>
__global__ __launch_bounds__(64 * W) void k_wide(DpArgs A, const double2 *__restrict__ lut_g,
                                                 const int32_t *__restrict__ list,
                                                 const int32_t *__restrict__ budget,
                                                 const int32_t *__restrict__ count)
{
    constexpr int R = MPB_WIDE_R;
    __shared__ double s_edge[W][2][64];
    __shared__ double s_acc[W];
    __shared__ int s_found[W];
    const int tid = threadIdx.x, w = tid >> 6, lane = tid & 63;
    for (int k = tid; k < 256; k += 64 * W) mpb_s_lut[k] = lut_g[k];
    __syncthreads();
    const int nlist = gload(count);
    int keep = lane == 0 ? 0 : -1;
    asm volatile("" : "+v"(keep));
    const double thr = A.prm.thr;
    for (int k = blockIdx.x; k < nlist; k += gridDim.x) {
        const int idx = gload(list + k);
        const int li = A.len ? clamp_len(gload(A.len + idx), A.prm.max_len) : A.prm.fixed_len;
        const int rows = FINAL ? li + 1 : gload(budget + k);
        const int nw = max(1, min(MPB_WIDE_WAVES, (rows + 64 * R - 1) / (64 * R)));
        if (nw > W || (W > 2 && nw <= W / 2)) continue;
        const int nblk = (li + 63) >> 6;
        const uint8_t *row = A.q + (int64_t)idx * A.stride;

        double v[R];
#pragma unroll
        for (int r = 0; r < R; r++) v[r] = 0.0;
        if (tid == 0) v[0] = 1.0;

        uint32_t curb = 0, nxtb = 0;
        const int nsteps = nblk + nw - 1;
        for (int s = 0; s < nsteps; s++) {
            const int t = s - w;
            if (w < nw && t >= 0 && t < nblk) {
                if (t == 0) curb = (lane < li) ? (uint32_t)gload(row + lane) : 0u;
                const int nb0 = (t + 1) * 64 + lane;
                nxtb = (nb0 < li) ? (uint32_t)gload(row + nb0) : 0u;
                __builtin_amdgcn_sched_barrier(0);
                const double *ein = &s_edge[w > 0 ? w - 1 : 0][(s + 1) & 1][0];
                double *eout = &s_edge[w][s & 1][0];
#pragma unroll 1
                for (int kb = 0; kb < 64; kb += 4) {
#pragma unroll
                    for (int tt = 0; tt < 4; tt++) {
                        const uint32_t byte = (uint32_t)__builtin_amdgcn_readlane((int)curb, kb + tt);
                        const double2 ab = mpb_s_lut[byte];
                        const double top = v[R - 1];
                        double cin = dpp_prev_row(top, keep);
                        if (w > 0) {
                            const double e = ein[kb + tt];
                            cin = lane == 0 ? e : cin;
                        }
                        if (lane == 63) eout[kb + tt] = top;
#pragma unroll
                        for (int r = R - 1; r >= 1; r--) v[r] = cell<false>(ab.x, v[r], ab.y, v[r - 1]);
                        v[0] = cell<false>(ab.x, v[0], ab.y, cin);
                    }
                }
                curb = nxtb;
            }
            __syncthreads();
        }

        for (int ww = 0; ww < nw; ww++) {
            if (w == ww) {
                const double acc0 = ww ? s_acc[ww - 1] : 0.0;
                const int found0 = ww ? s_found[ww - 1] : 0;
                double acc = acc0;
                int found = found0;
                if (!found0) {
                    double acc_in_mine = 0.0;
                    bool mine = false;
#pragma unroll 1
                    for (int g = 0; g < 64; g++) {
                        double acc_s = acc0;
                        int found_s = 0;
                        if (g > 0) {
                            acc_s = __shfl(acc, g - 1);
                            found_s = __shfl(found, g - 1);
                        }
                        if (lane == g) {
                            double a = acc_s;
#pragma unroll
                            for (int r = 0; r < R; r++) a = a + v[r];
                            const bool cross = !found_s && (a > thr);
                            mine = cross;
                            acc_in_mine = acc_s;
                            acc = a;
                            found = found_s | (cross ? 1 : 0);
                        }
                    }
                    if (mine) {
                        double lo = 0.0, hi = 0.0;
                        const int js = cdf_cross(v, acc_in_mine, thr, w * 64 * R + lane * R, lo, hi);
                        wide_report(A, idx, li, true, js, lo, hi);
                    }
                }
                if (lane == 63) { s_acc[ww] = acc; s_found[ww] = found; }
            }
            __syncthreads();
        }
        if (tid == 0 && !s_found[nw - 1]) {
            if (FINAL) {
                wide_report(A, idx, li, false, -1, 0.0, 0.0);
            } else {
                const int pos = atomicAdd(A.ovf_count, 1);
                A.ovf_list[pos] = idx;
            }
        }
        __syncthreads();
    }
}

template <bool FMA, bool SYS, typename PrmFn>
__device__ __forceinline__ bool small_one_read(const DpArgs &args, const DpArgs *s_args, PrmFn get_prm, const int li,
                                               const int64_t i, const int lane, int32_t *__restrict__ ns_out,
                                               uint8_t *__restrict__ cls_out, int32_t *__restrict__ ident,
                                               uint8_t *__restrict__ stage, const float2 *s_tab)
{
    f32x2 a01 = {0.f, 0.f};
    float s3 = 0.f;
    uint4 yr = make_uint4(0, 0, 0, 0);
    for (int c0 = 0; c0 * 16 < li; c0 += 64) {
        const int nv = li - (c0 + lane) * 16;
        if (nv > 0) {
            const uint8_t *src = args.q + i * args.stride + (int64_t)(c0 + lane) * 16;
            uint4 y;
            if (SYS) {
                const unsigned long long lo = __hip_atomic_load((const unsigned long long *)src, __ATOMIC_RELAXED, __HIP_MEMORY_SCOPE_SYSTEM);
                const unsigned long long hi = __hip_atomic_load((const unsigned long long *)src + 1, __ATOMIC_RELAXED, __HIP_MEMORY_SCOPE_SYSTEM);
                y = make_uint4((uint32_t)lo, (uint32_t)(lo >> 32), (uint32_t)hi, (uint32_t)(hi >> 32));
            } else {
                y = *reinterpret_cast<const uint4 *>(src);
            }
            if (stage) *reinterpret_cast<uint4 *>(stage + i * args.stride + (int64_t)(c0 + lane) * 16) = y;
            if (SYS) yr = make_uint4(mask_dword(y.x, nv), mask_dword(y.y, nv - 4), mask_dword(y.z, nv - 8), mask_dword(y.w, nv - 12));
            y.x = fill_dword(y.x, nv); y.y = fill_dword(y.y, nv - 4);
            y.z = fill_dword(y.z, nv - 8); y.w = fill_dword(y.w, nv - 12);
            pre_chunk(s_tab, y, a01, s3);
        }
    }
    const float n255 = floorf(a01.y * (1.0f / MPB_MARK_LOWER));
    const float rem = a01.y - MPB_MARK_LOWER * n255;
    const float nzero_f = floorf(rem * (1.0f / MPB_MARK_UPPER));
    float mu = a01.x, var = rem - MPB_MARK_UPPER * nzero_f;
    float k3 = var - 2.0f * s3;
    uint32_t ambi = (uint32_t)nzero_f + ((uint32_t)n255 << 16);
#pragma unroll
    for (int off = 1; off <= 32; off <<= 1) {
        mu += __shfl_xor(mu, off);
        var += __shfl_xor(var, off);
        k3 += __shfl_xor(k3, off);
        ambi += __shfl_xor(ambi, off);
    }
    const int nzero = (int)(ambi & 0xffffu), n_lower = (int)(ambi >> 16);
    const MpbDevParams prm = get_prm();
    const float v = fmaxf(var, 1e-12f);
    const float x = mu + prm.z * sqrtf(v) + (k3 / v) * prm.zq;
    int rows = (int)floorf(fminf(x, 1e9f) + 0.5f) + 1;
    if (prm.flags & MPB_FLAG_TEST_UNDERPREDICT) rows = rows / 2;
    rows = max(min(rows, li - nzero - n_lower + 1), 1);
    if (rows > MPB_TILE_MAX_ROWS) {
        if (lane == 0) args.pass[i] = 2;
        return false;
    }
    if (SYS && !FMA && li <= 1024 && rows <= 64 && !(prm.flags & ~MPB_FLAG_ROUND)) {
        int keep = lane == 0 ? 0 : -1;
        asm volatile("" : "+v"(keep));
        double v1 = lane == 0 ? 1.0 : 0.0;
        const int nchunks = (li + 15) >> 4;
#pragma unroll 1
        for (int ck = 0; ck < nchunks; ck++) {
            const uint32_t wq[4] = {(uint32_t)__builtin_amdgcn_readlane((int)yr.x, ck), (uint32_t)__builtin_amdgcn_readlane((int)yr.y, ck),
                                    (uint32_t)__builtin_amdgcn_readlane((int)yr.z, ck), (uint32_t)__builtin_amdgcn_readlane((int)yr.w, ck)};
#pragma unroll
            for (int d = 0; d < 4; d++) {
#pragma unroll
                for (int t = 0; t < 4; t++) {
                    const double2 ab = mpb_s_lut[(wq[d] >> (8 * t)) & 0xffu];
                    const double cin = dpp_prev_row(v1, keep);
                    v1 = cell<false>(ab.x, v1, ab.y, cin);
                }
            }
        }
        const double thr = prm.thr;
        double acc = 0.0, lo = 0.0, hi = 0.0;
        int js = -1;
#pragma unroll 1
        for (int g = 0; g < 64 && js < 0; g++) {
            const long long bits = __double_as_longlong(v1);
            const double vg = __longlong_as_double(((long long)__builtin_amdgcn_readlane((int)(bits >> 32), g) << 32) |
                                                   (unsigned int)__builtin_amdgcn_readlane((int)bits, g));
            const double na = acc + vg;
            if (na > thr) { lo = acc; hi = na; js = g; }
            acc = na;
        }
        if (lane == 0) {
            const int nsv = nzero + n_lower;
            __hip_atomic_store(ns_out + i, nsv, __ATOMIC_RELAXED, __HIP_MEMORY_SCOPE_SYSTEM);
            if (js < 0) {
                __hip_atomic_store(args.pass + i, (uint8_t)2, __ATOMIC_RELAXED, __HIP_MEMORY_SCOPE_SYSTEM);
            } else {
                double e;
                const bool keep = read_result(prm, true, js, lo, hi, nsv, nzero > 0, li, e);
                __hip_atomic_store((unsigned long long *)(args.ee + i), (unsigned long long)__double_as_longlong(e), __ATOMIC_RELAXED, __HIP_MEMORY_SCOPE_SYSTEM);
                __hip_atomic_store(args.pass + i, (uint8_t)(keep ? 1 : 0), __ATOMIC_RELAXED, __HIP_MEMORY_SCOPE_SYSTEM);
            }
        }
        return true;
    }
    const int c = c_class_of_rows.t[rows];
    const int thin = rows <= 2 ? 0 : 31 - __builtin_clz(rows - 1);
    const bool settled = settled_by_chernoff(prm, mu, li);
    if (lane == 0) {
        ns_out[i] = nzero + n_lower;
        if (args.ns != ns_out) const_cast<int32_t *>(args.ns)[i] = nzero + n_lower;
        cls_out[i] = (uint8_t)((settled ? MPB_CLS_SETTLED : c) | (nzero > 0 ? 0x80 : 0));
        ident[i] = (int32_t)i;
        if (settled) { args.ee[i] = __builtin_inf(); args.pass[i] = 0; }
    }
    if (settled) return false;
    __builtin_amdgcn_fence(__ATOMIC_RELEASE, "workgroup");
    __builtin_amdgcn_fence(__ATOMIC_ACQUIRE, "workgroup");
    const int32_t *pc = ident + i;
    switch (thin) {
#define MPB_CASE(ID, RR, GG) case ID: dp_tiles<RR, GG, FMA>(s_args, pc, 1, 0, 1); break;
        MPB_THIN_CLASSES(MPB_CASE)
#undef MPB_CASE
    default: break;
    }
    return false;
}

__device__ __forceinline__ void small_tables(const double2 *__restrict__ lut_g, float2 *s_tab, const int tid0, const int nthreads)
{
    for (int tid = tid0; tid < 256; tid += nthreads) {
        mpb_s_lut[tid] = lut_g[tid];
        const bool amb = tid == 0 || tid == 255;
        float p = __builtin_amdgcn_exp2f(-0.33219281f * (float)tid);
        p = amb ? 0.0f : p;
        s_tab[tid] = make_float2(p, tid == 0 ? MPB_MARK_UPPER : tid == 255 ? MPB_MARK_LOWER : p * (1.0f - p));
    }
}

template <bool FMA>
__global__ __launch_bounds__(256, MPB_DP_WAVES_PER_EU) void k_small(DpArgs args, const double2 *__restrict__ lut_g,
                                                                    int64_t n, int32_t *__restrict__ ns_out,
                                                                    uint8_t *__restrict__ cls_out,
                                                                    int32_t *__restrict__ ident,
                                                                    uint8_t *__restrict__ stage,
                                                                    uint32_t *__restrict__ done, uint32_t token)
{
    __shared__ float2 s_tab[256];
    __shared__ DpArgs s_args;
    const int tid = threadIdx.x, w = tid >> 6, lane = tid & 63;
    small_tables(lut_g, s_tab, tid, 256);
    if (tid == 0) { s_args = args; if (stage) s_args.q = stage; }
    __syncthreads();
    const int64_t i = (int64_t)blockIdx.x * 4 + w;
    if (i >= n) return;
    const int li = args.len ? clamp_len(args.len[i], args.prm.max_len) : args.prm.fixed_len;
    (void)small_one_read<FMA, false>(args, &s_args, [&] { return args.prm; }, li, i, lane, ns_out, cls_out, ident, stage, s_tab);
    if (done) {
        __threadfence_system();
        __builtin_amdgcn_wave_barrier();
        if (lane == 0) __hip_atomic_store(done + i, token, __ATOMIC_RELEASE, __HIP_MEMORY_SCOPE_SYSTEM);
    }
}

__global__ __launch_bounds__(256, MPB_DP_WAVES_PER_EU) void k_serve(MpbServeBox box, const double2 *__restrict__ lut_g,
                                                                    uint32_t generation, unsigned long long lifetime_ticks)
{
    __shared__ float2 s_tab[256];
    __shared__ DpArgs s_args[1];
    const int lane = threadIdx.x;
    constexpr int w = 0;
    small_tables(lut_g, s_tab, lane, 64);
    __syncthreads();
    const int e = blockIdx.x;
    if (e < box.n_ent) {
// ... 653 lines not shown
    __syncthreads();
    uint32_t base = 0;
#pragma unroll
    for (int k = 0; k < 3; k++) base += k < w ? s_wave[k] : 0;
    __syncthreads();
    return base + incl - x;
}

__global__ __launch_bounds__(256) void k_rag_sort(const int32_t *__restrict__ len, int64_t n, int32_t max_len, int key_shift,
                                                  int32_t split, int32_t low_pct,
                                                  int2 *__restrict__ ord, int32_t *__restrict__ gpre,
                                                  unsigned long long *__restrict__ wsum)
{
    __shared__ __attribute__((aligned(16))) uint16_t s_cnt[8 * 256];
    __shared__ __attribute__((aligned(16))) uint16_t s_idx[2][MPB_RG_WIN];
    __shared__ __attribute__((aligned(16))) uint16_t s_len[MPB_RG_WIN];
    __shared__ uint32_t s_wave[4];
    const int tid = threadIdx.x, lane = tid & 63, w = tid >> 6;
    const int64_t w0 = (int64_t)blockIdx.x * MPB_RG_WIN;
    const int m = (int)min((int64_t)MPB_RG_WIN, n - w0);
#pragma unroll
    for (int k = 0; k < 16; k++) {
        const int i = k * 256 + tid;
        const int l = i < m ? len[w0 + i] : 0;
        s_len[i] = (uint16_t)((l < 0 || l > max_len) ? 0xffff : l);
    }
    __syncthreads();
    auto key_of = [key_shift](uint32_t l) { return l == 0xffffu ? 0u : ((l + 15u) >> 4) >> key_shift; };
    uint32_t el[16];
    {
        const u32x4 a = *reinterpret_cast<const u32x4 *>(s_len + 16 * tid), b = *reinterpret_cast<const u32x4 *>(s_len + 16 * tid + 8);
        const uint32_t ww[8] = {a.x, a.y, a.z, a.w, b.x, b.y, b.z, b.w};
#pragma unroll
        for (int e = 0; e < 8; e++) { el[2 * e] = key_of(ww[e] & 0xffffu); el[2 * e + 1] = key_of(ww[e] >> 16); }
    }
    const int mine = min(16, max(0, m - 16 * tid));
#pragma unroll
    for (int pass = 0; pass < 2; pass++) {
        if (pass == 1) {
            __syncthreads();
            const u32x4 a = *reinterpret_cast<const u32x4 *>(s_idx[0] + 16 * tid), b = *reinterpret_cast<const u32x4 *>(s_idx[0] + 16 * tid + 8);
            const uint32_t ww[8] = {a.x, a.y, a.z, a.w, b.x, b.y, b.z, b.w};
#pragma unroll
            for (int e = 0; e < 8; e++) { el[2 * e] = ww[e] & 0xffffu; el[2 * e + 1] = ww[e] >> 16; }
        }
        unsigned long long c_lo = 0, c_hi = 0;
#pragma unroll
        for (int r = 0; r < 16; r++) {
            const int d = pass == 0 ? (int)(el[r] & 7u) : (int)(el[r] >> 12);
            const unsigned long long inc = r < mine ? 1ull << (16 * (d & 3)) : 0ull;
            c_lo += (d & 4) ? 0ull : inc;
            c_hi += (d & 4) ? inc : 0ull;
        }
#pragma unroll
        for (int d = 0; d < 8; d++) s_cnt[d * 256 + tid] = (uint16_t)(((d & 4) ? c_hi : c_lo) >> (16 * (d & 3)));
        __syncthreads();
        u32x4 c4 = *reinterpret_cast<const u32x4 *>(s_cnt + 8 * tid);
        uint32_t cc[8] = {c4.x & 0xffffu, c4.x >> 16, c4.y & 0xffffu, c4.y >> 16, c4.z & 0xffffu, c4.z >> 16, c4.w & 0xffffu, c4.w >> 16};
        uint32_t sum = 0;
#pragma unroll
        for (int e = 0; e < 8; e++) sum += cc[e];
        uint32_t run = rg_block_excl_scan(sum, s_wave, tid);
#pragma unroll
        for (int e = 0; e < 8; e++) { const uint32_t c = cc[e]; cc[e] = run; run += c; }
        c4.x = cc[0] | (cc[1] << 16); c4.y = cc[2] | (cc[3] << 16); c4.z = cc[4] | (cc[5] << 16); c4.w = cc[6] | (cc[7] << 16);
        *reinterpret_cast<u32x4 *>(s_cnt + 8 * tid) = c4;
        __syncthreads();
        unsigned long long p_lo = 0, p_hi = 0;
#pragma unroll
        for (int d = 0; d < 8; d++) {
            const unsigned long long v = (unsigned long long)s_cnt[d * 256 + tid] << (16 * (d & 3));
            if (d & 4) p_hi |= v; else p_lo |= v;
        }
#pragma unroll
        for (int r = 0; r < 16; r++) {
            const int d = pass == 0 ? (int)(el[r] & 7u) : (int)(el[r] >> 12);
            const uint32_t pos = (uint32_t)(((d & 4) ? p_hi : p_lo) >> (16 * (d & 3))) & 0xffffu;
            const unsigned long long inc = 1ull << (16 * (d & 3));
            p_lo += (d & 4) ? 0ull : inc;
            p_hi += (d & 4) ? inc : 0ull;
            if (r < mine) s_idx[pass][pos] = (uint16_t)(pass == 0 ? (uint32_t)(16 * tid + r) | ((el[r] >> 3) << 12) : el[r] & 0xfffu);
        }
    }
    __syncthreads();
    for (int p = tid; p < m; p += 256) {
        const int i = s_idx[1][p];
        const uint32_t l = s_len[i];
        ord[w0 + p] = make_int2((int)(w0 + i), l == 0xffffu ? -1 : (int)l);
    }
    if (w == 0) {
        int c = 0;
        if (lane * 64 < m) {
            const uint32_t k = key_of(s_len[s_idx[1][min(m, lane * 64 + 64) - 1]]);
            const int chunks = (int)(key_shift ? ((k + 1) << key_shift) - 1 : k);
            c = rg_group_cost(chunks) * 8;
            if (chunks <= split) c = c * low_pct / 100;
        }
        int pre = c;
#pragma unroll
        for (int off = 1; off < 64; off <<= 1) {
            const int x = __shfl_up(pre, off);
            if (lane >= off) pre += x;
        }
        if (lane * 64 < m) gpre[(w0 >> 6) + lane] = pre;
        if (lane == 63) wsum[blockIdx.x] = (unsigned long long)pre;
    }
}

__global__ __launch_bounds__(1024) void k_rag_scan(const unsigned long long *__restrict__ wsum, int nwin,
                                                   unsigned long long *__restrict__ wpre)
{
    __shared__ unsigned long long s_sum[1024];
    const int tid = threadIdx.x;
    const int per = (nwin + 1023) / 1024;
    const int a = min(nwin, tid * per), b = min(nwin, a + per);
    unsigned long long sum = 0;
    for (int k = a; k < b; k++) sum += wsum[k];
    s_sum[tid] = sum;
    __syncthreads();
    for (int off = 1; off < 1024; off <<= 1) {
        const unsigned long long x = tid >= off ? s_sum[tid - off] : 0;
        __syncthreads();
        s_sum[tid] += x;
        __syncthreads();
    }
    unsigned long long run = s_sum[tid] - sum;
    for (int k = a; k < b; k++) { wpre[k] = run; run += wsum[k]; }
    if (tid == 1023) wpre[nwin] = s_sum[1023];
}

__device__ __forceinline__ int rg_first_group(const unsigned long long *__restrict__ wpre, const int32_t *__restrict__ gpre,
                                              int nwin, int ngroups, int wv, int nwaves, int lane)
{
    if (wv >= nwaves) return ngroups;
    const unsigned long long T = wpre[nwin];
    const unsigned long long target = T * (unsigned long long)wv / (unsigned long long)nwaves;
    int lo = 0, hi = nwin;
    while (hi - lo > 1) {
        const int step = (hi - lo + 63) >> 6;
        const int idx = lo + lane * step;
        const bool ok = idx < hi && wpre[idx] <= target;
        const int k = __popcll(__ballot(ok)) - 1;
        lo += k * step;
        hi = min(hi, lo + step);
    }
    const unsigned long long rem = target - wpre[lo];
    const int ng = min(64, ngroups - lo * 64);
    const bool over = lane < ng && (unsigned long long)gpre[lo * 64 + lane] > rem;
    const unsigned long long m = __ballot(over);
    return lo * 64 + (m ? __builtin_ctzll(m) : ng - 1);
}

template <int R, int RLO>
__global__ __launch_bounds__(256, 4) void k_narrow_rg(const uint8_t *__restrict__ q, int64_t n, int64_t stride,
                                                   const int2 *__restrict__ ord, const unsigned long long *__restrict__ wpre,
                                                   const int32_t *__restrict__ gpre, int32_t *__restrict__ gstart, int32_t split,
                                                   MpbDevParams prm, const double2 *__restrict__ lut_g,
                                                   double *__restrict__ ee, int32_t *__restrict__ ns, uint8_t *__restrict__ pass,
                                                   int32_t *__restrict__ seg, int32_t *__restrict__ wave_count)
#include "mpb_narrow_rg.inc"

__global__ __launch_bounds__(256) void k_nar_compact(const int32_t *__restrict__ seg, const int32_t *__restrict__ wave_count,
                                                     int64_t nblk, int nwaves, int per_blk, const int32_t *__restrict__ gstart,
                                                     int32_t *__restrict__ list, int32_t *__restrict__ count)
{
    __shared__ int s_part[4];
    const int g = blockIdx.x, tid = threadIdx.x;
    int sum = 0;
    for (int k = tid; k < g; k += 256) sum += wave_count[k];
#pragma unroll
    for (int off = 32; off >= 1; off >>= 1) sum += __shfl_xor(sum, off);
    if ((tid & 63) == 0) s_part[tid >> 6] = sum;
    __syncthreads();
    const int off0 = s_part[0] + s_part[1] + s_part[2] + s_part[3];
    const int cnt = wave_count[g];
    const int32_t *src = gstart ? seg + 64 * (int64_t)gstart[g]
                                : seg + (int64_t)per_blk * ((int64_t)g * (nblk / nwaves) + min((int64_t)g, nblk % nwaves));
    int32_t *dst = list + off0;
    for (int k = tid; k < cnt; k += 256) dst[k] = src[k];
    if (g == nwaves - 1 && tid == 0) *count = off0 + cnt;
}

#undef MPB_NAR_AR
#undef MPB_NAR_RLO
#define MPB_NAR_AR MPB_AR_ODDS
#define MPB_NAR_RLO R
template <int R, int D>
__global__ __launch_bounds__(256) void k_odds_nar(const uint8_t *__restrict__ q, int64_t n, int64_t stride, int32_t li,
                                                  MpbDevParams prm, const double2 *__restrict__ lut_g,
                                                  double *__restrict__ ee, int32_t *__restrict__ ns, uint8_t *__restrict__ pass,
                                                  int32_t *__restrict__ seg, int32_t *__restrict__ wave_count)
#include "mpb_narrow_ring.inc"

template <int R, bool ALIGNED>
__global__ __launch_bounds__(256) void k_odds_nar_rs(const uint8_t *__restrict__ q, int64_t n, int64_t stride, int32_t li, int32_t k,
                                                     MpbDevParams prm, const double2 *__restrict__ lut_g,
                                                     double *__restrict__ ee, int32_t *__restrict__ ns, uint8_t *__restrict__ pass,
                                                     int32_t *__restrict__ seg, int32_t *__restrict__ wave_count)
#include "mpb_narrow_rs.inc"

template <int R>
__global__ __launch_bounds__(256, 4) void k_odds_nar_rg(const uint8_t *__restrict__ q, int64_t n, int64_t stride,
                                                   const int2 *__restrict__ ord, const unsigned long long *__restrict__ wpre,
                                                   const int32_t *__restrict__ gpre, int32_t *__restrict__ gstart, int32_t split,
                                                   MpbDevParams prm, const double2 *__restrict__ lut_g,
                                                   double *__restrict__ ee, int32_t *__restrict__ ns, uint8_t *__restrict__ pass,
                                                   int32_t *__restrict__ seg, int32_t *__restrict__ wave_count)
#include "mpb_narrow_rg.inc"
#undef MPB_NAR_RLO
#undef MPB_NAR_AR

__global__ __launch_bounds__(256) void k_sample(const uint8_t *__restrict__ q, int64_t n, int64_t stride, int32_t fixed_len,
                                                const int32_t *__restrict__ len, MpbDevParams prm, int n_sample,
                                                int32_t *__restrict__ hist)
{
    __shared__ float2 s_tab[256];
    __shared__ float4 s_pow[256];
    const int tid = threadIdx.x, w = tid >> 6, lane = tid & 63;
    {
        const bool amb = tid == 0 || tid == 255;
        float p = __builtin_amdgcn_exp2f(-0.33219281f * (float)tid);
        p = amb ? 0.0f : p;
        s_tab[tid] = make_float2(p, tid == 0 ? MPB_MARK_UPPER : tid == 255 ? MPB_MARK_LOWER : p * (1.0f - p));
        const float r = p / (1.0f - p);
        s_pow[tid] = make_float4(log1pf(-p), r, r * r, r * r * r);
    }
    __syncthreads();
    const int k = blockIdx.x * 4 + w;
    if (k >= n_sample) return;
    const int64_t step = n / n_sample;
    const int64_t i = min(n - 1, (int64_t)k * step + (int64_t)(mpb_mix64((uint64_t)k) % (uint64_t)step));
    const int li_raw = len ? len[i] : fixed_len;
    const bool bad_len = li_raw < 0 || li_raw > prm.max_len;
    const int li = bad_len ? 0 : li_raw;
    float mu = 0.f, var = 0.f, k3 = 0.f;
    float lp0 = 0.f, t1 = 0.f, t2 = 0.f, t3 = 0.f;
    int ambi = 0, lower = 0;
    for (int c0 = 0; c0 * 16 < li; c0 += 64 * 15) {
        f32x2 a01 = {0.f, 0.f};
        float s3 = 0.f;
        for (int c = c0 + lane; c * 16 < li && c < c0 + 64 * 15; c += 64) {
            uint4 y = *reinterpret_cast<const uint4 *>(q + i * stride + (int64_t)c * 16);
            const int nv = li - c * 16;
            y.x = fill_dword(y.x, nv); y.y = fill_dword(y.y, nv - 4);
            y.z = fill_dword(y.z, nv - 8); y.w = fill_dword(y.w, nv - 12);
            pre_chunk(s_tab, y, a01, s3);
            const uint32_t ww[4] = {y.x, y.y, y.z, y.w};
#pragma unroll
            for (int d = 0; d < 4; d++)
#pragma unroll
                for (int t = 0; t < 4; t++) {
                    const float4 e = s_pow[(ww[d] >> (8 * t)) & 0xffu];
                    lp0 += e.x; t1 += e.y; t2 += e.z; t3 += e.w;
                }
        }
        const float n255 = floorf(a01.y * (1.0f / MPB_MARK_LOWER));
        const float rem = a01.y - MPB_MARK_LOWER * n255;
        const float nzero = floorf(rem * (1.0f / MPB_MARK_UPPER));
        const float pvar = rem - MPB_MARK_UPPER * nzero;
        mu += a01.x; var += pvar; k3 += pvar - 2.0f * s3;
        ambi += (int)nzero + (int)n255;
        lower += (int)n255;
    }
#pragma unroll
    for (int off = 1; off <= 32; off <<= 1) {
        mu += __shfl_xor(mu, off); var += __shfl_xor(var, off);
        k3 += __shfl_xor(k3, off); ambi += __shfl_xor(ambi, off); lower += __shfl_xor(lower, off);
        lp0 += __shfl_xor(lp0, off); t1 += __shfl_xor(t1, off);
        t2 += __shfl_xor(t2, off); t3 += __shfl_xor(t3, off);
    }
    if (lane == 0) {
        const float vv = fmaxf(var, 1e-12f);
        const float x = mu + prm.z * sqrtf(vv) + (k3 / vv) * prm.zq;
        int rows = (int)floorf(fminf(x, 1e9f) + 0.5f) + 1;
        rows = max(rows, 5);
        const float thr = (float)prm.thr;
        const float p0 = __expf(lp0);
        const float e1 = t1, e2 = 0.5f * (t1 * t1 - t2), e3 = (t1 * t1 * t1 - 3.0f * t1 * t2 + 2.0f * t3) * (1.0f / 6.0f);
        float cdf = p0;
        if (cdf > thr) rows = 1;
        else if ((cdf += p0 * e1) > thr) rows = 2;
        else if ((cdf += p0 * e2) > thr) rows = 3;
        else if ((cdf += p0 * e3) > thr) rows = 4;
        rows = max(min(rows, li - ambi + 1), 1);
        atomicAdd(hist + ((lower > 0 || bad_len) ? 0 : min(rows, MPB_NAR_BUCKETS - 1)),
                  len ? max(1, (li + 15) >> 4) : 1);
        if (len && lower == 0 && !bad_len) {
            if (rows >= 3) atomicMin(hist + MPB_NAR_BUCKETS, (li + 15) >> 4);
            if (rows >= 4) atomicMin(hist + MPB_NAR_BUCKETS + 1, (li + 15) >> 4);
        }
    }
}

}

static inline int pre_blocks(int64_t n) { return (int)((n + MPB_PRE_READS - 1) / MPB_PRE_READS); }

void mpb_launch_prepass(const uint8_t *q, int64_t n, int64_t stride, const int32_t *len,
                        const MpbDevParams &prm, const MpbWorkspace &ws, int32_t *ns_out,
                        double *ee_out, uint8_t *pass_out, hipStream_t s, const int32_t *list)
{
#define MPB_PRE_LAUNCH(RG, LG, LS)                                                                                      \
    hipLaunchKernelGGL((k_prepass<RG, LG, LS>), dim3(pre_blocks(n)), dim3(256), 0, s, q, n, stride, len, prm, o, ws.blockhist, list)
    const PreOut o = {ws.cls, ns_out, ee_out, pass_out, ws.bad_len, ws.wide_list, ws.wide_rows, ws.wide_count};
    const bool long_rows = prm.max_len > 16 * 12 * MPB_PRE_NB;
    if (list) {
        if (len) { if (long_rows) MPB_PRE_LAUNCH(true, true, true); else MPB_PRE_LAUNCH(true, false, true); }
        else     { if (long_rows) MPB_PRE_LAUNCH(false, true, true); else MPB_PRE_LAUNCH(false, false, true); }
    } else {
        if (len) { if (long_rows) MPB_PRE_LAUNCH(true, true, false); else MPB_PRE_LAUNCH(true, false, false); }
        else     { if (long_rows) MPB_PRE_LAUNCH(false, true, false); else MPB_PRE_LAUNCH(false, false, false); }
    }
#undef MPB_PRE_LAUNCH
}

void mpb_launch_decode_classify(const uint8_t *seq, const uint8_t *qual, int32_t offset, uint8_t *out, int32_t *err,
                                int64_t n, int64_t stride, const int32_t *len, const MpbDevParams &prm,
                                const MpbWorkspace &ws, int32_t *ns_out, double *ee_out, uint8_t *pass_out, hipStream_t s)
{
    const PreOut o = {ws.cls, ns_out, ee_out, pass_out, ws.bad_len, ws.wide_list, ws.wide_rows, ws.wide_count};
    const PreDecode dec = {seq, qual, out, offset, err};
    const uint8_t *q = out;
    const uint32_t cpr = (uint32_t)(stride >> 4);
    const uint32_t magic = cpr == 1 ? 0u : (uint32_t)(((1ull << 32) + cpr - 1) / cpr);
    if (len) hipLaunchKernelGGL((k_classify_linear<true, true>), dim3(pre_blocks(n)), dim3(256), 0, s, q, n, stride, len, prm, o, ws.blockhist, dec, magic);
    else     hipLaunchKernelGGL((k_classify_linear<false, true>), dim3(pre_blocks(n)), dim3(256), 0, s, q, n, stride, len, prm, o, ws.blockhist, dec, magic);
}

void mpb_launch_encode(const uint8_t *q, int64_t n, int64_t stride, int32_t offset, uint8_t *seq, uint8_t *qual, hipStream_t s)
{
    const int64_t chunks = n * (stride / 16);
    hipLaunchKernelGGL(k_encode_ascii, dim3((unsigned)((chunks + 255) / 256)), dim3(256), 0, s, q, n, stride, offset, seq, qual);
}

void mpb_launch_scan(int64_t n, const int32_t *len, const MpbWorkspace &ws, hipStream_t s)
{
    const int nb = len ? MPB_LEN_BINS : 1;
    hipLaunchKernelGGL(k_scan, dim3(MPB_NCLS * nb), dim3(256), 0, s, ws.blockhist, pre_blocks(n), ws.tables);
    hipLaunchKernelGGL(k_tables, dim3(1), dim3(512), 0, s, ws.tables, nb, ws.ovf_count, ws.pass_count);
}

void mpb_launch_scatter(int64_t n, const int32_t *len, const int32_t *ns, const MpbDevParams &prm, const MpbWorkspace &ws,
                        hipStream_t s, const int32_t *list)
{
    if (len)
        hipLaunchKernelGGL((k_scatter<true>), dim3(pre_blocks(n)), dim3(256), 0, s, ws.cls, n, len, prm.max_len, prm.len_shift,
                           ws.blockhist, ws.tables, ns, ws.perm, ws.perm_ns, list);
    else
        hipLaunchKernelGGL((k_scatter<false>), dim3(pre_blocks(n)), dim3(256), 0, s, ws.cls, n, len, prm.max_len, prm.len_shift,
                           ws.blockhist, ws.tables, ns, ws.perm, ws.perm_ns, list);
}

#define MPB_DP_GRID (1 << 20)


static DpArgs make_args(const uint8_t *q, int64_t stride, const int32_t *len, const MpbDevParams &prm,
                        const MpbWorkspace &ws, const int32_t *ns, double *ee, uint8_t *pass, int final_pass)
{
    DpArgs A;
    A.q = q; A.stride = stride; A.len = len; A.ns = ns; A.cls = ws.cls; A.ee = ee; A.pass = pass;
    A.ovf_list = ws.ovf_list; A.ovf_count = ws.ovf_count; A.alg_cells = ws.alg_cells; A.prm = prm; A.final_pass = final_pass;
    A.perm = ws.perm; A.perm_ns = final_pass == 0 ? ws.perm_ns : nullptr;
    return A;
}

void mpb_launch_dp(const uint8_t *q, int64_t n, int64_t stride, const int32_t *len,
                   const MpbDevParams &prm, const MpbWorkspace &ws, const int32_t *ns,
                   double *ee, uint8_t *pass, hipStream_t s, const double2 *lut_odds)
{
    const int64_t tiles = (n + 63) / 64 + MPB_NCLS;
    const int chunk_tiles = tiles >= 32768 ? MPB_DP_CHUNK : tiles >= 16384 ? 4 : tiles >= 8192 ? 2 : 1;
    constexpr int grid_cap = MPB_DP_GRID;
    int64_t want = (tiles + 4 * chunk_tiles - 1) / (4 * chunk_tiles);
    const int blocks = (int)(want < grid_cap ? (want > 0 ? want : 1) : grid_cap);
    DpArgs A = make_args(q, stride, len, prm, ws, ns, ee, pass, 0);
    if (lut_odds)
        hipLaunchKernelGGL(k_dp_odds, dim3(blocks), dim3(256), 0, s, A, lut_odds, ws.tables, ws.perm, chunk_tiles);
    else if (prm.flags & MPB_FLAG_FAST_FMA)
        hipLaunchKernelGGL((k_dp<true, false>), dim3(blocks), dim3(256), 0, s, A, ws.lut, ws.tables, ws.perm, chunk_tiles);
    else
        hipLaunchKernelGGL((k_dp<false, false>), dim3(blocks), dim3(256), 0, s, A, ws.lut, ws.tables, ws.perm, chunk_tiles);
}

#define MPB_WIDE_GRID 1024

template <bool FINAL>
static void launch_wide(const DpArgs &A, const double2 *lut, const int32_t *list, const int32_t *budget,
                        const int32_t *count, int max_rows, hipStream_t s)
{
    const int max_waves = (max_rows + MPB_TILE_MAX_ROWS - 1) / MPB_TILE_MAX_ROWS;
    hipLaunchKernelGGL((k_wide<FINAL, 2>), dim3(MPB_WIDE_GRID), dim3(64 * 2), 0, s, A, lut, list, budget, count);
    if (max_waves > 2) hipLaunchKernelGGL((k_wide<FINAL, 4>), dim3(MPB_WIDE_GRID), dim3(64 * 4), 0, s, A, lut, list, budget, count);
    if (max_waves > 4) hipLaunchKernelGGL((k_wide<FINAL, 8>), dim3(MPB_WIDE_GRID), dim3(64 * 8), 0, s, A, lut, list, budget, count);
    if (max_waves > 8) hipLaunchKernelGGL((k_wide<FINAL, 16>), dim3(MPB_WIDE_GRID), dim3(64 * 16), 0, s, A, lut, list, budget, count);
}

void mpb_launch_wide(const uint8_t *q, int64_t stride, const int32_t *len, const MpbDevParams &prm,
                     const MpbWorkspace &ws, const int32_t *ns, double *ee, uint8_t *pass, hipStream_t s)
{
    DpArgs A = make_args(q, stride, len, prm, ws, ns, ee, pass, 0);
    A.perm_ns = nullptr;
    launch_wide<false>(A, ws.lut, ws.wide_list, ws.wide_rows, ws.wide_count, prm.max_len + 1, s);
}

void mpb_launch_overflow(const uint8_t *q, int64_t n, int64_t stride, const int32_t *len,
                         const MpbDevParams &prm, const MpbWorkspace &ws, const int32_t *ns,
                         double *ee, uint8_t *pass, hipStream_t s)
{
    (void)n;
    if (prm.max_len + 1 > MPB_TILE_MAX_ROWS) {
        hipLaunchKernelGGL(k_tables_overflow, dim3(1), dim3(64), 0, s, ws.tables2, ws.ovf_count, MPB_NCLS - 1, ws.ovf_total);
        DpArgs A = make_args(q, stride, len, prm, ws, ns, ee, pass, 1);
        launch_wide<true>(A, ws.lut, ws.ovf_list, nullptr, ws.ovf_count, prm.max_len + 1, s);
        return;
    }
    static const MpbClass classes[MPB_NCLS] = MPB_CLASS_TABLE;
    int wc = MPB_NCLS - 1;
    for (int c = MPB_NCLS - 1; c >= 0; c--)
        if (classes[c].cap >= prm.max_len + 1) wc = c;
    hipLaunchKernelGGL(k_tables_overflow, dim3(1), dim3(64), 0, s, ws.tables2, ws.ovf_count, wc, ws.ovf_total);
    DpArgs A = make_args(q, stride, len, prm, ws, ns, ee, pass, 1);
    const int blocks = 256;
    hipLaunchKernelGGL((k_dp<false, true>), dim3(blocks), dim3(256), 0, s, A, ws.lut, ws.tables2, ws.ovf_list, MPB_DP_CHUNK);
}

void mpb_launch_lambda(const uint8_t *q, int64_t n, int64_t stride, const int32_t *len, int32_t fixed_len,
                       const double2 *lut_ap, double *lambda, int32_t *ns, int32_t *bad, hipStream_t s)
{
    int64_t blocks = (n + 255) / 256;
    if (blocks > (1 << 20)) blocks = 1 << 20;
    if (len)
        hipLaunchKernelGGL((k_lambda<true>), dim3((unsigned)blocks), dim3(256), 0, s, q, n, stride, len,
                           fixed_len, lut_ap, lambda, ns, bad);
    else
        hipLaunchKernelGGL((k_lambda<false>), dim3((unsigned)blocks), dim3(256), 0, s, q, n, stride, len,
                           fixed_len, lut_ap, lambda, ns, bad);
}

void mpb_launch_poisson_tail(const double *lambda, const int32_t *ns, const int32_t *len, int64_t n, const MpbDevParams &prm,
                             double *ee, uint8_t *pass, int32_t *handed, MpbPoissonRec *rec, int32_t rec_cap,
                             unsigned long long *n_pass, hipStream_t s)
{
    int64_t blocks = (n + 255) / 256;
    if (blocks > 2048) blocks = 2048;
    if (blocks < 1) blocks = 1;
    hipLaunchKernelGGL(k_poisson_tail, dim3((unsigned)blocks), dim3(256), 0, s, lambda, ns, len, n, prm, ee, pass, handed, rec,
                       rec_cap, n_pass);
}

void mpb_launch_poisson_patch(const MpbPoissonFix *fix, int32_t m, double *ee, uint8_t *pass, hipStream_t s)
{
    if (m <= 0) return;
    hipLaunchKernelGGL(k_poisson_patch, dim3((unsigned)((m + 255) / 256)), dim3(256), 0, s, fix, m, ee, pass);
}

void mpb_launch_decode(const uint8_t *seq, const uint8_t *qual, int64_t n, int64_t stride, const int32_t *len,
                       int32_t fixed_len, int32_t offset, uint8_t *out, int32_t *err, hipStream_t s)
{
    const int64_t chunks = n * (stride / 16);
    hipLaunchKernelGGL(k_decode_ascii, dim3((unsigned)((chunks + 255) / 256)), dim3(256), 0, s, seq, qual, n,
                       stride, len, fixed_len, offset, out, err);
}

void mpb_launch_pack_text(const uint8_t *text, int64_t text_bytes, const mpb_text_row *rows, int64_t n, int64_t k0, int32_t offset,
                          bool lower_n_is_base, int64_t stride, uint8_t *out, int32_t *len_out, uint8_t *flags_out,
                          int64_t *status, hipStream_t s)
{
    int64_t blocks = (n + 31) / 32;
    if (blocks > (1 << 20)) blocks = 1 << 20;
    if (blocks < 1) blocks = 1;
    if (lower_n_is_base)
        hipLaunchKernelGGL((k_pack_text<true>), dim3((unsigned)blocks), dim3(256), 0, s, text, text_bytes, rows, n, k0, offset, stride, out,
                           len_out, flags_out, (long long *)status);
    else
        hipLaunchKernelGGL((k_pack_text<false>), dim3((unsigned)blocks), dim3(256), 0, s, text, text_bytes, rows, n, k0, offset, stride, out,
                           len_out, flags_out, (long long *)status);
}

void mpb_launch_count(const uint8_t *pass, int64_t n, const MpbWorkspace &ws, hipStream_t s)
{
    int blocks = (int)((n + 255) / 256);
    if (blocks > 1024) blocks = 1024;
    if (blocks < 1) blocks = 1;
    hipLaunchKernelGGL(k_count, dim3(blocks), dim3(256), 0, s, pass, n, ws.pass_count);
}

void mpb_launch_synth(uint8_t *q, int64_t n, int64_t stride, int32_t fixed_len, int32_t min_len,
                      int32_t max_len, int32_t *len, uint64_t seed, int64_t first_read,
                      hipStream_t s, int32_t profile)
{
    const int64_t chunks = n * (stride / 16);
    const int64_t blocks = (chunks + 255) / 256;
    hipLaunchKernelGGL(k_synth, dim3((unsigned)blocks), dim3(256), 0, s, q, n, stride, fixed_len,
                       min_len, max_len, len, seed, first_read, profile);
}

void mpb_launch_small(const uint8_t *q, int64_t n, int64_t stride, const int32_t *len, const MpbDevParams &prm,
                      const MpbWorkspace &ws, int32_t *ns, double *ee, uint8_t *pass, hipStream_t s, const MpbSmallHost *host)
{
    DpArgs A = make_args(q, stride, len, prm, ws, host && host->ns_dev ? host->ns_dev : ns, ee, pass, 2);
    const int blocks = (int)((n + 3) / 4);
    uint8_t *stage = host ? host->stage : nullptr;
    uint32_t *done = host ? host->done : nullptr;
    const uint32_t token = host ? host->token : 0u;
    if (prm.flags & MPB_FLAG_FAST_FMA)
        hipLaunchKernelGGL((k_small<true>), dim3(blocks), dim3(256), 0, s, A, ws.lut, n, ns, ws.cls, ws.perm, stage, done, token);
    else
        hipLaunchKernelGGL((k_small<false>), dim3(blocks), dim3(256), 0, s, A, ws.lut, n, ns, ws.cls, ws.perm, stage, done, token);
}

void mpb_launch_serve(const MpbServeBox &box, const double2 *lut, uint32_t generation, uint32_t lifetime_ms, hipStream_t s)
{
    (void)hipMemsetAsync(box.gone, 0, sizeof(uint32_t), s);
    hipLaunchKernelGGL(k_serve, dim3(box.n_ent), dim3(64), 0, s, box, lut, generation, (unsigned long long)lifetime_ms * 100000ull);
}

static int nar_rs_reads_per_lane(int64_t stride, int rows0)
{
    if (stride % 16 != 0 || stride > (1 << 16)) return 0;
    if (stride % 64 != 0 && rows0 != 2) return 0;
    int k = 1;
    while ((k * stride) % 128 != 0) k *= 2;
    return k;
}

static int mpb_narrow_rg_key_shift(int64_t stride)
{
    int ks = 0;
    while (((stride >> 4) >> ks) >= MPB_RG_BINS) ks++;
    return ks;
}

static decltype(&k_narrow_rg<2, 2>) const nar_rg_forms[MPB_NRG_EXACT_FORMS] = {k_narrow_rg<2, 2>, k_narrow_rg<3, 3>, k_narrow_rg<4, 4>,
                                                                                k_narrow_rg<3, 2>, k_narrow_rg<4, 3>};
static decltype(&k_odds_nar_rg<2>) const nar_rg_odds_forms[MPB_NRG_FORMS - MPB_NRG_EXACT_FORMS] = {k_odds_nar_rg<2>, k_odds_nar_rg<3>,
                                                                                                     k_odds_nar_rg<4>};

void mpb_narrow_rg_blocks_per_cu(int per_cu[MPB_NRG_FORMS])
{
    for (int f = 0; f < MPB_NRG_FORMS; f++) {
        int nb = 0;
        const void *const form = f < MPB_NRG_EXACT_FORMS ? (const void *)nar_rg_forms[f] : (const void *)nar_rg_odds_forms[f - MPB_NRG_EXACT_FORMS];
        if (hipOccupancyMaxActiveBlocksPerMultiprocessor(&nb, form, 256, 0) != hipSuccess || nb < 1) {
            (void)hipGetLastError();
            nb = 1;
        }
        per_cu[f] = nb;
    }
}

static int64_t nar_grid_blocks(int64_t nblk, int n_cu, int per_cu, int grid_cap, int *waves)
{
    int64_t blocks = (nblk + 3) / 4;
    if (blocks > (int64_t)n_cu * per_cu) blocks = (int64_t)n_cu * per_cu;
    if (blocks > MPB_NAR_MAX_WAVES / 4) blocks = MPB_NAR_MAX_WAVES / 4;
    if (grid_cap > 0 && blocks > grid_cap) blocks = grid_cap;
    if (blocks < 1) blocks = 1;
    *waves = (int)blocks * 4;
    return blocks;
}

static void launch_narrow_odds(int rows0, const double2 *lut, const uint8_t *q, int64_t n, int64_t stride, int32_t fixed_len,
                               const int32_t *len, const MpbDevParams &prm, const MpbWorkspace &ws, double *ee, int32_t *ns, uint8_t *pass,
                               int n_cu, const int *rg_per_cu, int grid_cap, int *waves, hipStream_t s)
{
    const int ri = rows0 <= 2 ? 0 : rows0 == 3 ? 1 : 2;
    const int rg = MPB_NRG_EXACT_FORMS + ri;
    const int rs_k = len ? 0 : nar_rs_reads_per_lane(stride, rows0);
    const int lds = len || rs_k ? 256 * (int)sizeof(nar_entry_t) + 4 * MPB_NRS_TILE
                                : 256 * (int)sizeof(nar_entry_t) + MPB_NAR_DEPTH * 4 * MPB_NAR_PANEL + 32;
    int per_cu = (160 * 1024) / lds;
    if (len && rg_per_cu[rg] < per_cu) per_cu = rg_per_cu[rg];
    const int per_blk = 64 * (rs_k ? rs_k : 1);
    const int64_t nblk = (n + per_blk - 1) / per_blk;
    const int64_t blocks = nar_grid_blocks(nblk, n_cu, per_cu, grid_cap, waves);
    const int nwaves = (int)blocks * 4;
    const dim3 grid((unsigned)blocks), block(256);
    if (len) {
        const int64_t nwin = (n + MPB_RG_WIN - 1) / MPB_RG_WIN;
        hipLaunchKernelGGL(k_rag_sort, dim3((unsigned)nwin), dim3(256), 0, s, len, n, prm.max_len, mpb_narrow_rg_key_shift(stride),
                           -1, 100, ws.rg_ord, ws.rg_gpre, ws.rg_wsum);
        hipLaunchKernelGGL(k_rag_scan, dim3(1), dim3(1024), 0, s, ws.rg_wsum, (int)nwin, ws.rg_wpre);
        hipLaunchKernelGGL(nar_rg_odds_forms[ri], grid, block, 0, s, q, n, stride, ws.rg_ord, ws.rg_wpre, ws.rg_gpre, ws.rg_gstart,
                           -1, prm, lut, ee, ns, pass, ws.nar_seg, ws.nar_wave_count);
    } else if (rs_k) {
        static decltype(&k_odds_nar_rs<2, true>) const forms[4] = {k_odds_nar_rs<2, true>, k_odds_nar_rs<3, true>, k_odds_nar_rs<4, true>,
                                                                   k_odds_nar_rs<2, false>};
        hipLaunchKernelGGL(forms[stride % 64 != 0 ? 3 : ri], grid, block, 0, s, q, n, stride, fixed_len, rs_k, prm, lut, ee, ns, pass,
                           ws.nar_seg, ws.nar_wave_count);
    } else {
        static decltype(&k_odds_nar<2, MPB_NAR_DEPTH>) const forms[3] = {k_odds_nar<2, MPB_NAR_DEPTH>, k_odds_nar<3, MPB_NAR_DEPTH>,
                                                                         k_odds_nar<4, MPB_NAR_DEPTH>};
        hipLaunchKernelGGL(forms[ri], grid, block, 0, s, q, n, stride, fixed_len, prm, lut, ee, ns, pass, ws.nar_seg, ws.nar_wave_count);
    }
    hipLaunchKernelGGL(k_nar_compact, dim3((unsigned)nwaves), dim3(256), 0, s, ws.nar_seg, ws.nar_wave_count, nblk, nwaves, per_blk,
                       len ? (const int32_t *)ws.rg_gstart : nullptr, ws.nar_list, ws.nar_count);
}

void mpb_launch_narrow(int rows0, int split_chunks, const uint8_t *q, int64_t n, int64_t stride, int32_t fixed_len, const int32_t *len,
                       const MpbDevParams &prm, const MpbWorkspace &ws, double *ee, int32_t *ns, uint8_t *pass, int n_cu,
                       const int *rg_per_cu, int grid_cap, int *waves, hipStream_t s, const double2 *lut_odds)
{
    if (lut_odds) return launch_narrow_odds(rows0, lut_odds, q, n, stride, fixed_len, len, prm, ws, ee, ns, pass, n_cu, rg_per_cu, grid_cap, waves, s);
    const int ri = rows0 <= 2 ? 0 : rows0 == 3 ? 1 : 2;
    const bool mixed = len && split_chunks > 0 && rows0 >= 3;
    const int rg = mixed ? ri + 2 : ri;
    const int rs_k = len ? 0 : nar_rs_reads_per_lane(stride, rows0);
    const int lds = len || rs_k ? 256 * (int)sizeof(nar_entry_t) + 4 * MPB_NRS_TILE
                                : 256 * (int)sizeof(nar_entry_t) + MPB_NAR_DEPTH * 4 * MPB_NAR_PANEL + 32;
    int per_cu = (160 * 1024) / lds;
    if (len && rg_per_cu[rg] < per_cu) per_cu = rg_per_cu[rg];
    const int per_blk = 64 * (rs_k ? rs_k : 1);
    const int64_t nblk = (n + per_blk - 1) / per_blk;
    const int64_t blocks = nar_grid_blocks(nblk, n_cu, per_cu, grid_cap, waves);
    const int nwaves = (int)blocks * 4;
    const dim3 grid((unsigned)blocks), block(256);
    if (len) {
        const int64_t nwin = (n + MPB_RG_WIN - 1) / MPB_RG_WIN;
        hipLaunchKernelGGL(k_rag_sort, dim3((unsigned)nwin), dim3(256), 0, s, len, n, prm.max_len, mpb_narrow_rg_key_shift(stride),
                           mixed ? split_chunks : -1, rows0 >= 4 ? 80 : 86, ws.rg_ord, ws.rg_gpre, ws.rg_wsum);
        hipLaunchKernelGGL(k_rag_scan, dim3(1), dim3(1024), 0, s, ws.rg_wsum, (int)nwin, ws.rg_wpre);
        hipLaunchKernelGGL(nar_rg_forms[rg], grid, block, 0, s, q, n, stride, ws.rg_ord, ws.rg_wpre, ws.rg_gpre, ws.rg_gstart,
                           split_chunks, prm, ws.lut, ee, ns, pass, ws.nar_seg, ws.nar_wave_count);
    } else if (rs_k) {
        static decltype(&k_narrow_rs<2, true>) const forms[4] = {k_narrow_rs<2, true>, k_narrow_rs<3, true>, k_narrow_rs<4, true>,
                                                                 k_narrow_rs<2, false>};
        hipLaunchKernelGGL(forms[stride % 64 != 0 ? 3 : ri], grid, block, 0, s, q, n, stride, fixed_len, rs_k, prm, ws.lut, ee, ns, pass,
                           ws.nar_seg, ws.nar_wave_count);
    } else {
        static decltype(&k_narrow<2, MPB_NAR_DEPTH>) const forms[3] = {k_narrow<2, MPB_NAR_DEPTH>, k_narrow<3, MPB_NAR_DEPTH>,
                                                                       k_narrow<4, MPB_NAR_DEPTH>};
        hipLaunchKernelGGL(forms[ri], grid, block, 0, s, q, n, stride, fixed_len, prm, ws.lut, ee, ns, pass, ws.nar_seg, ws.nar_wave_count);
    }
    hipLaunchKernelGGL(k_nar_compact, dim3((unsigned)nwaves), dim3(256), 0, s, ws.nar_seg, ws.nar_wave_count, nblk, nwaves, per_blk,
                       len ? (const int32_t *)ws.rg_gstart : nullptr, ws.nar_list, ws.nar_count);
}

void mpb_launch_sample(const uint8_t *q, int64_t n, int64_t stride, int32_t fixed_len, const int32_t *len, const MpbDevParams &prm,
                       const MpbWorkspace &ws, int n_sample, hipStream_t s)
{
    (void)hipMemsetAsync(ws.nar_sample, 0, MPB_NAR_BUCKETS * sizeof(int32_t), s);
    (void)hipMemsetAsync(ws.nar_sample + MPB_NAR_BUCKETS, 0x7f, 2 * sizeof(int32_t), s);
    hipLaunchKernelGGL(k_sample, dim3((unsigned)((n_sample + 3) / 4)), dim3(256), 0, s, q, n, stride, fixed_len, len, prm, n_sample, ws.nar_sample);
}
```

### moira_amd/csrc/mpb_resident.cpp

```cpp

#include "mpb_ctx.h"

#include <cmath>
#include <cstdlib>
#include <cstring>


MpbDevParams make_dev_params(const mpb_filter_params *p, int32_t fixed_len, int32_t max_len)
{
    MpbDevParams d;
    d.thr = 1 - p->alpha;
    d.uncert = p->uncert;
    d.maxerrors = p->maxerrors;
    const double z = inv_norm_cdf(1 - p->alpha);
    d.z = (float)z;
    d.zq = (float)((z * z - 1) / 6);
    if (!(z == z) || std::isinf(z)) { d.z = 1e30f; d.zq = 0.0f; }
    d.clow = (float)(sqrt(2 * log(1 / (1 - p->alpha))) * 1.0001);
    d.ambig_mode = p->ambig_mode;
    d.flags = p->flags;
    d.fixed_len = fixed_len;
    d.max_len = max_len;
    d.len_shift = MPB_LEN_SHIFT;
    while (((max_len - 1) >> d.len_shift) >= MPB_LEN_BINS) d.len_shift++;
    return d;
}

static int check_device_batch(const void *d_q, int64_t n, int64_t row_stride, const int32_t *d_len, int32_t fixed_len,
                              const void *d_ee, const void *d_ns, const void *d_pass, int32_t *max_len_out)
{
    if (n < 0) return fail(MPB_E_INVALID, "n < 0");
    if (n > 0x7fffffffll - 4096) return fail(MPB_E_INVALID, "batch of %lld reads exceeds 2^31; split it", (long long)n);
    if (row_stride <= 0 || row_stride % 16 != 0) return fail(MPB_E_INVALID, "row_stride must be a positive multiple of 16");
    if (row_stride > MPB_MAX_STRIDE) return fail(MPB_E_INVALID, "row_stride %lld exceeds %d (reads longer than %d bases are not supported)", (long long)row_stride, MPB_MAX_STRIDE, MPB_MAX_LEN);
    if (((uintptr_t)d_q & 15) != 0) return fail(MPB_E_INVALID, "quality matrix must be 16-byte aligned");
    if (!d_len && (fixed_len < 0 || fixed_len > row_stride)) return fail(MPB_E_INVALID, "fixed_len %d does not fit row_stride %lld", fixed_len, (long long)row_stride);
    const int32_t max_len = d_len ? (int32_t)(row_stride < MPB_MAX_LEN ? row_stride : MPB_MAX_LEN) : fixed_len;
    if (max_len > MPB_MAX_LEN)
        return fail(MPB_E_INVALID, "reads longer than %d bases are not supported", MPB_MAX_LEN);
    if (n > 0 && (!d_q || !d_ee || !d_ns || !d_pass)) return fail(MPB_E_INVALID, "NULL device buffer");
    *max_len_out = max_len;
    return MPB_OK;
}

static int prepare_batch(mpb_ctx *c, int64_t n, int32_t max_len)
{
    int rc = ensure_workspace(c, n);
    if (rc) return rc;
    if (max_len + 1 > MPB_TILE_MAX_ROWS) {
        if ((rc = ensure_wide_workspace(c, n))) return rc;
        HIPCHK(hipMemsetAsync(c->ws.wide_count, 0, sizeof(int32_t), c->stream));
    }
    return MPB_OK;
}

static int fetch_counts(mpb_ctx *c, int64_t n, int64_t row_stride, const int32_t *d_len, int32_t max_len, const uint8_t *d_pass,
                        bool sorted, mpb_filter_counts *counts)
{
    hipStream_t s = c->stream;
    unsigned long long *np = &c->pin->n_pass;
    int32_t *novf = &c->pin->n_overflow, *bad = &c->pin->bad_len;
    *novf = *bad = 0;
    if (!sorted) HIPCHK(hipMemsetAsync(c->ws.pass_count, 0, sizeof(unsigned long long), s));
    mpb_launch_count(d_pass, n, c->ws, s);
    HIPCHK(hipMemcpyAsync(np, c->ws.pass_count, sizeof(*np), hipMemcpyDeviceToHost, s));
    if (sorted) HIPCHK(hipMemcpyAsync(novf, c->ws.ovf_count, sizeof(*novf), hipMemcpyDeviceToHost, s));
    if (d_len) HIPCHK(hipMemcpyAsync(bad, c->ws.bad_len, sizeof(*bad), hipMemcpyDeviceToHost, s));
    HIPCHK(hipStreamSynchronize(s));
    if (*bad) {
        HIPCHK(hipMemsetAsync(c->ws.bad_len, 0, sizeof(int32_t), s));
        return fail(MPB_E_INVALID, "%d read length(s) in d_len outside 0..%d (row_stride %lld; reads longer than %d bases "
                    "are not supported); those reads were given ee = NaN, pass = 0", *bad, max_len, (long long)row_stride, MPB_MAX_LEN);
    }
    counts->n_pass = (int64_t)*np;
    counts->n_fail = n - (int64_t)*np;
    counts->n_overflow = *novf;
    return MPB_OK;
}

static int filter_device_tail(mpb_ctx *c, const uint8_t *d_q, int64_t n, int64_t row_stride, const int32_t *d_len,
                              const MpbDevParams &prm, double *d_ee, int32_t *d_ns, uint8_t *d_pass, mpb_filter_counts *counts,
                              const int32_t *d_list = nullptr)
{
    hipStream_t s = c->stream;
    const int32_t max_len = prm.max_len;
    { Span t(c, MPB_K_SCAN);     mpb_launch_scan(n, d_len, c->ws, s); }
    { Span t(c, MPB_K_SCATTER);  mpb_launch_scatter(n, d_len, d_ns, prm, c->ws, s, d_list); }
    const double2 *lut_odds = (prm.flags & MPB_FLAG_ODDS) && c->ws.lut == c->d_lut ? c->d_lut_odds : nullptr;
    { Span t(c, MPB_K_DP);       mpb_launch_dp(d_q, n, row_stride, d_len, prm, c->ws, d_ns, d_ee, d_pass, s, lut_odds); }
    if (max_len + 1 > MPB_TILE_MAX_ROWS) { Span t(c, MPB_K_WIDE); mpb_launch_wide(d_q, row_stride, d_len, prm, c->ws, d_ns, d_ee, d_pass, s); }
    { Span t(c, MPB_K_OVERFLOW); mpb_launch_overflow(d_q, n, row_stride, d_len, prm, c->ws, d_ns, d_ee, d_pass, s); }
    HIPCHK(hipGetLastError());
    return counts ? fetch_counts(c, n, row_stride, d_len, max_len, d_pass, true, counts) : MPB_OK;
}

static bool narrow_eligible(const mpb_ctx *c, int64_t n, int64_t row_stride, const int32_t *d_len, int32_t fixed_len, const mpb_filter_params *p)
{
    uint32_t forbidden = MPB_FLAG_FAST_FMA | MPB_FLAG_ODDS | MPB_FLAG_TEST_UNDERPREDICT | MPB_FLAG_DECISION_ONLY | MPB_FLAG_COUNT_CELLS | MPB_FLAG_NO_NARROW;
    if (p->flags & MPB_FLAG_ODDS_NARROW) forbidden &= ~MPB_FLAG_ODDS;
    if (!(c->narrow_ok && n >= 1 && !(p->flags & forbidden) && c->ws.lut == c->d_lut)) return false;
    return d_len ? row_stride <= MPB_RG_MAX_STRIDE : fixed_len >= 1;
}

static int filter_device_general(mpb_ctx *c, const uint8_t *d_q, int64_t n, int64_t row_stride, const int32_t *d_len,
                                 int32_t fixed_len, int32_t max_len, const mpb_filter_params *params,
                                 double *d_ee, int32_t *d_ns, uint8_t *d_pass, mpb_filter_counts *counts,
                                 const int32_t *d_list = nullptr, int64_t n_matrix = 0)
{
    int rc;
    if ((rc = prepare_batch(c, d_list && n_matrix > n ? n_matrix : n, max_len))) return rc;
    const MpbDevParams prm = make_dev_params(params, fixed_len, max_len);
    if (params->flags & MPB_FLAG_COUNT_CELLS) HIPCHK(hipMemsetAsync(c->ws.alg_cells, 0, sizeof(unsigned long long), c->stream));
    { Span t(c, MPB_K_PREPASS);  mpb_launch_prepass(d_q, n, row_stride, d_len, prm, c->ws, d_ns, d_ee, d_pass, c->stream, d_list); }
    return filter_device_tail(c, d_q, n, row_stride, d_len, prm, d_ee, d_ns, d_pass, counts, d_list);
}

static int narrow_choose(mpb_ctx *c, const uint8_t *d_q, int64_t n, int64_t row_stride, const int32_t *d_len, int32_t fixed_len,
                         const mpb_filter_params *params, const MpbDevParams &prm, int *rows0, int *split)
{
    *rows0 = 0;
    *split = 0;
    c->last_path.sampled = 0;
    const int forced = (int)((params->flags >> 8) & 15u);
    if (forced) {
        *rows0 = forced < MPB_NAR_MIN_ROWS ? MPB_NAR_MIN_ROWS : forced > MPB_NAR_MAX_ROWS ? MPB_NAR_MAX_ROWS : forced;
        *split = d_len && !(params->flags & MPB_FLAG_ODDS_NARROW) ? (int)((params->flags >> 12) & 255u) : 0;
        return MPB_OK;
    }
    if (n < MPB_NAR_AUTO_MIN_READS) return MPB_OK;
    auto &ch = c->nar_choice;
    if (d_len) fixed_len = -1;
    const bool same = ch.valid && ch.n == n && ch.stride == row_stride && ch.fixed_len == fixed_len &&
                      memcmp(&ch.alpha, &params->alpha, sizeof(double)) == 0 && ch.flags == params->flags;
    if (same && ch.calls < 64) { ch.calls++; *rows0 = ch.rows0; *split = ch.split; return MPB_OK; }
    int n_sample = (int)(n / 1024 < 256 ? 256 : n / 1024 > 4096 ? 4096 : n / 1024);
    { Span t(c, MPB_K_SAMPLE); mpb_launch_sample(d_q, n, row_stride, fixed_len, d_len, prm, c->ws, n_sample, c->stream); }
    HIPCHK(hipMemcpyAsync(c->pin->sample, c->ws.nar_sample, sizeof(c->pin->sample), hipMemcpyDeviceToHost, c->stream));
    HIPCHK(hipStreamSynchronize(c->stream));
    c->last_path.sampled = 1;
    const int32_t *sample = c->pin->sample;
    int weight = 0;
    for (int k = 0; k < MPB_NAR_BUCKETS; k++) { c->last_path.sample_hist[k] = sample[k]; weight += sample[k]; }
    const bool odds = (params->flags & MPB_FLAG_ODDS_NARROW) != 0;
    *rows0 = narrow_rows_from_sample(sample, weight, odds);
    if (d_len && *rows0 >= 3 && !odds) {
        const int need = sample[MPB_NAR_BUCKETS + (*rows0 - 3)];
        if (need > 0 && need < (1 << 20)) {
            const int cut = need - 1 - need / 16;
            if (cut >= 4) *split = cut > 255 ? 255 : cut;
        }
    }
    ch.split = *split;
    {
        double back = sample[0];
        for (int r = *rows0 + 1; r < MPB_NAR_BUCKETS; r++) back += sample[r];
        ch.expect_back = weight > 0 ? back / weight : 0.0;
    }
    ch.valid = true; ch.n = n; ch.stride = row_stride; ch.fixed_len = fixed_len; ch.alpha = params->alpha; ch.flags = params->flags;
    ch.rows0 = *rows0; ch.calls = 0;
    return MPB_OK;
}

static int narrow_grid_cap()
{
    const char *e = getenv("MPB_NARROW_GRID_BLOCKS");
    if (!e || !*e) return 0;
    char *end = nullptr;
    const long v = strtol(e, &end, 10);
    return *end == 0 && v >= 1 && v <= MPB_NAR_GRID_CAP_MAX ? (int)v : 0;
}

static int filter_device_narrow(mpb_ctx *c, int rows0, int split, const uint8_t *d_q, int64_t n, int64_t row_stride, const int32_t *d_len,
                                int32_t fixed_len, const mpb_filter_params *params, const MpbDevParams &prm,
                                double *d_ee, int32_t *d_ns, uint8_t *d_pass, mpb_filter_counts *counts)
{
    int rc;
    hipStream_t s = c->stream;
    if ((rc = ensure_narrow_workspace(c, n, d_len != nullptr))) return rc;
    const int grid_cap = narrow_grid_cap();
    int nwaves = 0;
    { Span t(c, MPB_K_NARROW);
      mpb_launch_narrow(rows0, split, d_q, n, row_stride, fixed_len, d_len, prm, c->ws, d_ee, d_ns, d_pass, c->n_cu > 0 ? c->n_cu : 256,
                        c->rg_per_cu, grid_cap, &nwaves, s, (params->flags & MPB_FLAG_ODDS_NARROW) ? c->d_lut_odds : nullptr); }
    HIPCHK(hipGetLastError());
    HIPCHK(hipMemcpyAsync(&c->pin->nar_count, c->ws.nar_count, sizeof(int32_t), hipMemcpyDeviceToHost, s));
    HIPCHK(hipStreamSynchronize(s));
    const int64_t m = c->pin->nar_count;
    c->last_path.narrow_rows = rows0;
    c->last_path.narrow_waves = nwaves;
    c->last_path.narrow_split = d_len && rows0 >= 3 ? split : 0;
    c->last_path.n_fallback = m;
    const bool forced = ((params->flags >> 8) & 15u) != 0;
    if (!forced && m > n / 2) c->nar_choice.valid = false;
    if (!forced && split > 0 && (double)m > (1.5 * c->nar_choice.expect_back + 0.002) * (double)n) c->nar_choice.split = 0;
    c->classes_whole = false;
    if (m > 0) {
        if (!forced && m > n / 2) {
            c->last_path.n_fallback = n;
            c->classes_whole = true;
            return filter_device_general(c, d_q, n, row_stride, d_len, fixed_len, prm.max_len, params, d_ee, d_ns, d_pass, counts);
        }
        mpb_filter_params sub = *params;
        sub.flags = (sub.flags & ~((15u << 8) | (255u << 12) | MPB_FLAG_ODDS_NARROW)) | MPB_FLAG_NO_NARROW;
        if ((rc = filter_device_general(c, d_q, m, row_stride, d_len, fixed_len, prm.max_len, &sub, d_ee, d_ns, d_pass, nullptr, c->ws.nar_list, n))) return rc;
        HIPCHK(hipGetLastError());
    }
    return counts ? fetch_counts(c, n, row_stride, d_len, prm.max_len, d_pass, m > 0, counts) : MPB_OK;
}

int mpb_filter_device(mpb_ctx *c, const uint8_t *d_q, int64_t n, int64_t row_stride,
                      const int32_t *d_len, int32_t fixed_len, const mpb_filter_params *params,
                      double *d_ee, int32_t *d_ns, uint8_t *d_pass, mpb_filter_counts *counts)
{
    CTXCHK(c);
    int rc = check_params(params);
    if (rc) return rc;
    int32_t max_len = 0;
    if ((rc = check_device_batch(d_q, n, row_stride, d_len, fixed_len, d_ee, d_ns, d_pass, &max_len))) return rc;
    if (counts) { counts->n_reads = n; counts->n_pass = 0; counts->n_fail = 0; counts->n_overflow = 0; }
    if (n == 0) return MPB_OK;
    c->classified.valid = false;
    c->last_path = mpb_path_info{};
    c->classes_whole = true;
    if ((rc = ensure_workspace(c, 1))) return rc;
    if (narrow_eligible(c, n, row_stride, d_len, fixed_len, params)) {
        const MpbDevParams prm = make_dev_params(params, fixed_len, max_len);
        int rows0 = 0, split = 0;
        if ((rc = narrow_choose(c, d_q, n, row_stride, d_len, fixed_len, params, prm, &rows0, &split))) return rc;
        if (rows0) return filter_device_narrow(c, rows0, split, d_q, n, row_stride, d_len, fixed_len, params, prm, d_ee, d_ns, d_pass, counts);
    }
    return filter_device_general(c, d_q, n, row_stride, d_len, fixed_len, max_len, params, d_ee, d_ns, d_pass, counts);
}

int mpb_last_path(mpb_ctx *c, mpb_path_info *out)
{
    CTXCHK(c);
    if (!out) return fail(MPB_E_INVALID, "NULL output");
    *out = c->last_path;
    return MPB_OK;
}

int mpb_last_algorithmic_cells(mpb_ctx *c, int64_t *cells)
{
    CTXCHK(c);
    if (!cells) return fail(MPB_E_INVALID, "NULL output");
    if (!c->ws_small.p) { *cells = 0; return MPB_OK; }
    unsigned long long v = 0;
    int rc = copy_sync(c, &v, c->ws.alg_cells, sizeof(v), hipMemcpyDeviceToHost);
    if (rc) return rc;
    *cells = (int64_t)v;
    return MPB_OK;
}


int mpb_decode_classify_device(mpb_ctx *c, const uint8_t *d_seq, const uint8_t *d_qual, int64_t n, int64_t row_stride,
                               const int32_t *d_len, int32_t fixed_len, int32_t fastq_offset,
                               const mpb_filter_params *params, uint8_t *d_q_out, double *d_ee, int32_t *d_ns,
                               uint8_t *d_pass, int32_t *d_err)
{
    CTXCHK(c);
    int rc = check_params(params);
    if (rc) return rc;
    int32_t max_len = 0;
    if ((rc = check_device_batch(d_q_out, n, row_stride, d_len, fixed_len, d_ee, d_ns, d_pass, &max_len))) return rc;
    if ((((uintptr_t)d_seq | (uintptr_t)d_qual) & 15) != 0) return fail(MPB_E_INVALID, "matrices must be 16-byte aligned");
    if (n > 0 && (!d_seq || !d_qual)) return fail(MPB_E_INVALID, "NULL device buffer");
    if (row_stride > MPB_SMALL_MAX_STRIDE)
        return fail(MPB_E_INVALID, "row_stride %lld: the classify-at-source pass takes rows of up to %d bytes (decode with "
                    "mpb_decode_ascii_device, then mpb_filter_device)", (long long)row_stride, MPB_SMALL_MAX_STRIDE);
    c->classified.valid = false;
    if (n == 0) return MPB_OK;
    if ((rc = prepare_batch(c, n, max_len))) return rc;
    const MpbDevParams prm = make_dev_params(params, fixed_len, max_len);
    { Span t(c, MPB_K_PREPASS);
      mpb_launch_decode_classify(d_seq, d_qual, fastq_offset, d_q_out, d_err, n, row_stride, d_len, prm, c->ws, d_ns, d_ee, d_pass, c->stream); }
    HIPCHK(hipGetLastError());
    c->classified = {true, d_q_out, n, row_stride, d_len, fixed_len, *params, d_ee, d_ns, d_pass};
    return MPB_OK;
}

int mpb_filter_device_classified(mpb_ctx *c, const uint8_t *d_q, int64_t n, int64_t row_stride,
                                 const int32_t *d_len, int32_t fixed_len, const mpb_filter_params *params,
                                 double *d_ee, int32_t *d_ns, uint8_t *d_pass, mpb_filter_counts *counts)
{
    CTXCHK(c);
    int rc = check_params(params);
    if (rc) return rc;
    int32_t max_len = 0;
    if ((rc = check_device_batch(d_q, n, row_stride, d_len, fixed_len, d_ee, d_ns, d_pass, &max_len))) return rc;
    if (counts) { counts->n_reads = n; counts->n_pass = 0; counts->n_fail = 0; counts->n_overflow = 0; }
    if (n == 0) return MPB_OK;
    const auto &k = c->classified;
    const bool same_params = k.valid && memcmp(&k.params.alpha, &params->alpha, sizeof(double)) == 0 &&
                             memcmp(&k.params.uncert, &params->uncert, sizeof(double)) == 0 &&
                             memcmp(&k.params.maxerrors, &params->maxerrors, sizeof(double)) == 0 &&
                             k.params.ambig_mode == params->ambig_mode && k.params.flags == params->flags;
    if (!same_params || k.q != d_q || k.n != n || k.stride != row_stride || k.len != d_len || k.fixed_len != fixed_len ||
        k.ee != d_ee || k.ns != d_ns || k.pass != d_pass)
        return fail(MPB_E_INVALID, "mpb_filter_device_classified: the last call on this context that classified a batch "
                                   "(mpb_decode_classify_device) did not produce THIS batch with THESE parameters and result arrays");
    c->classified.valid = false;
    c->classes_whole = true;
    const MpbDevParams prm = make_dev_params(params, fixed_len, max_len);
    return filter_device_tail(c, d_q, n, row_stride, d_len, prm, d_ee, d_ns, d_pass, counts);
}

int mpb_encode_ascii_device(mpb_ctx *c, const uint8_t *d_q, int64_t n, int64_t row_stride, int32_t fastq_offset,
                            uint8_t *d_seq_out, uint8_t *d_qual_out)
{
    CTXCHK(c);
    if (n < 0 || row_stride <= 0 || row_stride % 16 != 0) return fail(MPB_E_INVALID, "bad matrix shape");
    if ((((uintptr_t)d_q | (uintptr_t)d_seq_out | (uintptr_t)d_qual_out) & 15) != 0) return fail(MPB_E_INVALID, "matrices must be 16-byte aligned");
    if (n == 0) return MPB_OK;
    if (!d_q || !d_seq_out || !d_qual_out) return fail(MPB_E_INVALID, "NULL device buffer");
    if (n * (row_stride / 16) / 256 > 0x7fffffffll) return fail(MPB_E_INVALID, "too large for one launch; split it");
    mpb_launch_encode(d_q, n, row_stride, fastq_offset, d_seq_out, d_qual_out, c->stream);
    HIPCHK(hipGetLastError());
    return MPB_OK;
}

int mpb_last_class_histogram(mpb_ctx *c, int32_t *caps, int64_t *cnts, int32_t max_classes)
{
    CTXCHK(c);
    if (!caps || !cnts || max_classes < 0) return fail(MPB_E_INVALID, "bad arguments");
    if (!c->classes_whole)
        return fail(MPB_E_INVALID, "the last filter call took the narrow pass (%d rows): there is no class histogram of its batch; "
                                   "call with MPB_FLAG_NO_NARROW to get one", c->last_path.narrow_rows);
    if (!c->ws.tables) return 0;
    static const MpbClass classes[MPB_NCLS] = MPB_CLASS_TABLE;
    MpbTables h;
    int rc = copy_sync(c, &h, c->ws.tables, sizeof(h), hipMemcpyDeviceToHost);
    if (rc) return rc;
    int k = 0;
    for (; k < MPB_NCLS && k < max_classes; k++) { caps[k] = classes[k].cap; cnts[k] = h.count[k]; }
    return k;
}

int mpb_last_read_budgets(mpb_ctx *c, int32_t *caps_out, int64_t n)
{
    CTXCHK(c);
    if (!caps_out || n < 0) return fail(MPB_E_INVALID, "bad arguments");
    if (!c->classes_whole)
        return fail(MPB_E_INVALID, "the last filter call took the narrow pass (%d rows): there are no per-read row budgets of its "
                                   "batch; call with MPB_FLAG_NO_NARROW to get them", c->last_path.narrow_rows);
    if (n > c->ws_cap || !c->ws.cls) return fail(MPB_E_INVALID, "no filter call of at least %lld reads precedes", (long long)n);
    static const MpbClass classes[MPB_NCLS] = MPB_CLASS_TABLE;
    std::vector<uint8_t> cls((size_t)n);
    int rc = copy_sync(c, cls.data(), c->ws.cls, (size_t)n, hipMemcpyDeviceToHost);
    if (rc) return rc;
    for (int64_t i = 0; i < n; i++) {
        const int k = cls[(size_t)i] & 0x7f;
        caps_out[i] = k < MPB_NCLS ? classes[k].cap : 0;
    }
    return MPB_OK;
}

int mpb_decode_ascii_device(mpb_ctx *c, const uint8_t *d_seq, const uint8_t *d_qual, int64_t n, int64_t row_stride,
                            const int32_t *d_len, int32_t fixed_len, int32_t fastq_offset, uint8_t *d_out, int32_t *d_err)
{
    CTXCHK(c);
    if (n < 0 || row_stride <= 0 || row_stride % 16 != 0) return fail(MPB_E_INVALID, "bad matrix shape");
    if ((((uintptr_t)d_seq | (uintptr_t)d_qual | (uintptr_t)d_out) & 15) != 0) return fail(MPB_E_INVALID, "matrices must be 16-byte aligned");
    if (!d_len && (fixed_len < 0 || fixed_len > row_stride)) return fail(MPB_E_INVALID, "fixed_len does not fit row_stride");
    if (n == 0) return MPB_OK;
    if (!d_seq || !d_qual || !d_out) return fail(MPB_E_INVALID, "NULL device buffer");
    if (n * (row_stride / 16) / 256 > 0x7fffffffll) return fail(MPB_E_INVALID, "too large for one launch; split it");
    mpb_launch_decode(d_seq, d_qual, n, row_stride, d_len, fixed_len, fastq_offset, d_out, d_err, c->stream);
    HIPCHK(hipGetLastError());
    return MPB_OK;
}

int mpb_synth_fill_device(mpb_ctx *c, uint8_t *d_q, int64_t n, int64_t row_stride, int32_t fixed_len,
                          int32_t min_len, int32_t max_len, int32_t *d_len, uint64_t seed, int64_t first_read)
{
    return mpb_synth_fill_device_profile(c, d_q, n, row_stride, fixed_len, min_len, max_len, d_len, seed, first_read, 0);
}

int mpb_synth_fill_device_profile(mpb_ctx *c, uint8_t *d_q, int64_t n, int64_t row_stride, int32_t fixed_len,
                                  int32_t min_len, int32_t max_len, int32_t *d_len, uint64_t seed, int64_t first_read,
                                  int32_t profile)
{
    CTXCHK(c);
    if (profile != 0 && profile != 1) return fail(MPB_E_INVALID, "unknown synthetic profile %d", profile);
    if (n < 0 || row_stride <= 0 || row_stride % 16 != 0) return fail(MPB_E_INVALID, "bad matrix shape");
    if (fixed_len > 0) { if (fixed_len > row_stride) return fail(MPB_E_INVALID, "fixed_len exceeds row_stride"); }
    else if (min_len < 1 || max_len < min_len || max_len > row_stride || !d_len)
        return fail(MPB_E_INVALID, "ragged fill needs 1 <= min_len <= max_len <= row_stride and d_len");
    if (n == 0) return MPB_OK;
    if (n * (row_stride / 16) / 256 > 0x7fffffffll) return fail(MPB_E_INVALID, "fill too large for one launch; split it");
    mpb_launch_synth(d_q, n, row_stride, fixed_len, min_len, max_len, d_len, seed, first_read, c->stream, profile);
    HIPCHK(hipGetLastError());
    return MPB_OK;
}
```

Baseline: 2.630 billion reads/s.

## Precompute per-read class ranks in prepass and fuse scan with table build

The prepass now computes each read's rank within its class key using wave ballots and stores it in a new rank array, replacing shared-memory atomics for the block histogram. A new ranked scatter kernel uses these ranks to place reads directly into the permutation without re-ranking. The separate table-building launch is folded into the last block of the scan via a ticket counter, and the overflow-tables kernel is folded into the overflow DP launch. This cuts kernel launches and scatter work, at the cost of an extra uint16 rank array and more complex prepass logic.

Result: no change. 2.670 billion reads/s (median of 6 runs) (+1.5%).

```diff
diff --git a/moira_amd/csrc/mpb_context.cpp b/moira_amd/csrc/mpb_context.cpp
--- a/moira_amd/csrc/mpb_context.cpp
+++ b/moira_amd/csrc/mpb_context.cpp
@@ -226,6 +226,7 @@
         c->ws.tables = &b->tables;
         c->ws.tables2 = &b->tables2;
         c->ws.ovf_count = &b->ovf_count;
+        c->ws.scan_ticket = &b->scan_ticket;
         c->ws.bad_len = &b->bad_len;
         c->ws.pass_count = &b->pass_count;
         c->ws.ovf_total = &b->ovf_total;
@@ -243,6 +244,7 @@
     MpbWorkspace &w = c->ws;
     int rc = carve(c, c->ws_block, [&w, cap, nb](Carver &k) {
         k.take(w.cls, cap);
+        k.take(w.rank, cap);
         k.take(w.perm, cap + (int64_t)MPB_NCLS * 64);
         k.take(w.perm_ns, cap + (int64_t)MPB_NCLS * 64);
         k.take(w.blockhist, nb * MPB_SKEYS);
diff --git a/moira_amd/csrc/mpb_ctx.h b/moira_amd/csrc/mpb_ctx.h
--- a/moira_amd/csrc/mpb_ctx.h
+++ b/moira_amd/csrc/mpb_ctx.h
@@ -71,6 +71,7 @@
     alignas(256) MpbTables tables;
     alignas(256) MpbTables tables2;
     alignas(64) int32_t ovf_count;
+    alignas(64) uint32_t scan_ticket;
     alignas(64) int32_t bad_len;
     alignas(64) unsigned long long pass_count;
     alignas(64) long long ovf_total;
diff --git a/moira_amd/csrc/mpb_internal.h b/moira_amd/csrc/mpb_internal.h
--- a/moira_amd/csrc/mpb_internal.h
+++ b/moira_amd/csrc/mpb_internal.h
@@ -65,6 +65,7 @@
 
 struct MpbWorkspace {
     uint8_t  *cls;
+    uint16_t *rank;
     int32_t  *perm;
     uint16_t *perm_ns;
     int32_t  *blockhist;
@@ -72,6 +73,7 @@
     MpbTables *tables2;
     int32_t  *ovf_list;
     int32_t  *ovf_count;
+    uint32_t *scan_ticket;
     int32_t  *bad_len;
     long long *ovf_total;
     int32_t  *wide_list;
@@ -134,7 +136,7 @@
 void mpb_launch_serve(const MpbServeBox &box, const double2 *lut, uint32_t generation, uint32_t lifetime_ms, hipStream_t s);
 void mpb_launch_scan(int64_t n, const int32_t *len, const MpbWorkspace &ws, hipStream_t s);
 void mpb_launch_scatter(int64_t n, const int32_t *len, const int32_t *ns, const MpbDevParams &prm, const MpbWorkspace &ws,
-                        hipStream_t s, const int32_t *list = nullptr);
+                        hipStream_t s, const int32_t *list = nullptr, bool ranked = false);
 void mpb_launch_dp(const uint8_t *q, int64_t n, int64_t stride, const int32_t *len,
                    const MpbDevParams &prm, const MpbWorkspace &ws, const int32_t *ns,
                    double *ee, uint8_t *pass, hipStream_t s, const double2 *lut_odds = nullptr);
diff --git a/moira_amd/csrc/mpb_kernels.hip b/moira_amd/csrc/mpb_kernels.hip
--- a/moira_amd/csrc/mpb_kernels.hip
+++ b/moira_amd/csrc/mpb_kernels.hip
@@ -180,9 +180,34 @@
 struct PreOut {
     uint8_t *cls; int32_t *ns; double *ee; uint8_t *pass;
     int32_t *bad_len, *wide_list, *wide_rows, *wide_count;
+    uint16_t *rank;
 };
 
-__device__ __forceinline__ void class_read(int64_t i, float mu, float var, float k3, uint32_t ambi, int li, bool bad, bool ragged,
+#define MPB_RANK_SLOTS (4 * MPB_PRE_ROUNDS)
+#define MPB_RANK_NONE 0xffffu
+
+template <int BITS>
+__device__ __forceinline__ int wave_rank(int kk, uint8_t *s_cnt, int slot)
+{
+    unsigned long long m = __ballot(kk >= 0);
+#pragma unroll
+    for (int b = 0; b < BITS; b++) {
+        const bool bit = (kk >> b) & 1;
+        const unsigned long long set = __ballot(bit);
+        m &= bit ? set : ~set;
+    }
+    const int rank = (int)__builtin_amdgcn_mbcnt_hi((uint32_t)(m >> 32), __builtin_amdgcn_mbcnt_lo((uint32_t)m, 0u));
+    if (kk >= 0 && rank == 0) s_cnt[kk * MPB_RANK_SLOTS + slot] = (uint8_t)__popcll(m);
+    return rank;
+}
+
+__device__ __forceinline__ uint32_t byte_sum(uint32_t x)
+{
+    x = (x & 0x00ff00ffu) + ((x >> 8) & 0x00ff00ffu);
+    return (x & 0xffffu) + (x >> 16);
+}
+
+__device__ __forceinline__ int class_read(int64_t i, float mu, float var, float k3, uint32_t ambi, int li, bool bad, bool ragged,
                                            const MpbDevParams &prm, const PreOut &o, int *s_hist, int nb)
 {
     const int nzero = (int)(ambi & 0xffffu), n255 = (int)(ambi >> 16);
@@ -219,8 +244,11 @@
         o.cls[i] = (uint8_t)(MPB_CLS_WIDE | (nzero > 0 ? 0x80 : 0));
     } else {
         o.cls[i] = (uint8_t)(c | (nzero > 0 ? 0x80 : 0));
-        atomicAdd(&s_hist[c * nb + (ragged ? min(MPB_LEN_BINS - 1, li >> prm.len_shift) : 0)], 1);
-    }
+        const int key = c * nb + (ragged ? min(MPB_LEN_BINS - 1, li >> prm.len_shift) : 0);
+        if (s_hist) atomicAdd(&s_hist[key], 1);
+        return key;
+    }
+    return -1;
 }
 
 template <bool RAGGED, bool LONG, bool LISTED>
@@ -231,7 +259,9 @@
 {
     __shared__ float2 s_tab[256];
     __shared__ float4 s_row[4][64];
-    __shared__ int s_hist[RAGGED ? MPB_SKEYS : MPB_NCLS];
+    __shared__ uint4 s_cnt[RAGGED ? MPB_SKEYS : MPB_NCLS];
+    __shared__ uint16_t s_rk[MPB_PRE_READS];
+    static_assert(MPB_RANK_SLOTS == 16 && MPB_SKEYS <= 512 && MPB_NCLS <= 32, "a key's counts are one uint4; a key has 9 bits (5: one bin)");
     const int32_t *__restrict__ len = RAGGED ? len_arg : nullptr;
     constexpr int nb = RAGGED ? MPB_LEN_BINS : 1;
     const int tid = threadIdx.x, w = tid >> 6, lane = tid & 63;
@@ -241,7 +271,9 @@
         p = amb ? 0.0f : p;
         s_tab[tid] = make_float2(p, tid == 0 ? MPB_MARK_UPPER : tid == 255 ? MPB_MARK_LOWER : p * (1.0f - p));
     }
-    for (int k = tid; k < MPB_NCLS * nb; k += 256) s_hist[k] = 0;
+    for (int k = tid; k < MPB_NCLS * nb; k += 256) s_cnt[k] = make_uint4(0, 0, 0, 0);
+#pragma unroll
+    for (int round = 0; round < MPB_PRE_ROUNDS; round++) s_rk[round * 256 + tid] = (uint16_t)MPB_RANK_NONE;
     __syncthreads();
 
     const int r16 = lane & 15, cl = lane >> 4;
@@ -328,17 +360,37 @@
     wave_lds_fence();
     {
         const int64_t k = wave_row0 + lane;
+        int kk = -1;
         if (k < n) {
             const int64_t i = LISTED ? (int64_t)list[k] : k;
             const float4 e = s_row[w][lane];
             const int li = len ? clamp_len(len[i], prm.max_len) : prm.fixed_len;
-            class_read(i, e.x, e.y, e.z, __float_as_uint(e.w), li, RAGGED && li != len[i], RAGGED, prm, o, s_hist, nb);
-        }
+            kk = class_read(i, e.x, e.y, e.z, __float_as_uint(e.w), li, RAGGED && li != len[i], RAGGED, prm, o, nullptr, nb);
+        }
+        const int rank = wave_rank<RAGGED ? 9 : 5>(kk, reinterpret_cast<uint8_t *>(s_cnt), round * 4 + w);
+        if (kk >= 0) s_rk[round * 256 + tid] = (uint16_t)(kk << 6 | rank);
     }
     wave_lds_fence();
     }
     __syncthreads();
-    for (int k = tid; k < MPB_NCLS * nb; k += 256) blockhist[(int64_t)k * gridDim.x + blockIdx.x] = s_hist[k];
+    for (int k = tid; k < MPB_NCLS * nb; k += 256) {
+        const uint4 c = s_cnt[k];
+        blockhist[(int64_t)k * gridDim.x + blockIdx.x] = (int32_t)(byte_sum(c.x) + byte_sum(c.y) + byte_sum(c.z) + byte_sum(c.w));
+    }
+#pragma unroll
+    for (int round = 0; round < MPB_PRE_ROUNDS; round++) {
+        const uint32_t rk = s_rk[round * 256 + tid];
+        if (rk == MPB_RANK_NONE) continue;
+        const int64_t k = (int64_t)blockIdx.x * MPB_PRE_READS + round * 256 + tid;
+        const int64_t i = LISTED ? (int64_t)list[k] : k;
+        const uint4 c = s_cnt[rk >> 6];
+        const uint32_t cw[4] = {c.x, c.y, c.z, c.w};
+        uint32_t before = byte_sum(cw[round] & ((1u << (8 * w)) - 1u));
+#pragma unroll
+        for (int r = 0; r < MPB_PRE_ROUNDS; r++)
+            if (r < round) before += byte_sum(cw[r]);
+        o.rank[i] = (uint16_t)(before + (rk & 63u));
+    }
 }
 
 #define MPB_LIN_K 5
@@ -458,39 +510,12 @@
     for (int k = tid; k < MPB_NCLS * nb; k += 256) blockhist[(int64_t)k * gridDim.x + blockIdx.x] = s_hist[k];
 }
 
-__global__ __launch_bounds__(256) void k_scan(int32_t *__restrict__ blockhist, int nblocks,
-                                              MpbTables *__restrict__ tb)
-{
-    __shared__ int s_part[256];
-    const int c = blockIdx.x, tid = threadIdx.x;
-    const int seg = (nblocks + 255) / 256;
-    const int b0 = tid * seg, b1 = min(nblocks, b0 + seg);
-    int sum = 0;
-    int32_t *bh = blockhist + (int64_t)c * nblocks;
-    for (int b = b0; b < b1; b++) sum += bh[b];
-    s_part[tid] = sum;
-    __syncthreads();
-    for (int off = 1; off < 256; off <<= 1) {
-        int v = (tid >= off) ? s_part[tid - off] : 0;
-        __syncthreads();
-        s_part[tid] += v;
-        __syncthreads();
-    }
-    int run = s_part[tid] - sum;
-    for (int b = b0; b < b1; b++) {
-        const int h = bh[b];
-        bh[b] = run;
-        run += h;
-    }
-    if (tid == 255) tb->kcount[c] = s_part[255];
-}
-
-__global__ __launch_bounds__(512) void k_tables(MpbTables *__restrict__ tb, int nb, int32_t *__restrict__ ovf_count,
-                                                unsigned long long *__restrict__ pass_count)
+__device__ __forceinline__ void build_tables(MpbTables *__restrict__ tb, int nb, int32_t *__restrict__ ovf_count,
+                                             unsigned long long *__restrict__ pass_count)
 {
     __shared__ int s_k[MPB_SKEYS], s_cnt[MPB_NCLS], s_base[MPB_NCLS + 1], s_tile[MPB_NCLS + 1];
     const int tid = threadIdx.x;
-    for (int k = tid; k < MPB_NCLS * nb; k += 512) s_k[k] = tb->kcount[k];
+    for (int k = tid; k < MPB_NCLS * nb; k += 256) s_k[k] = __hip_atomic_load(&tb->kcount[k], __ATOMIC_RELAXED, __HIP_MEMORY_SCOPE_AGENT);
     __syncthreads();
     if (tid < MPB_NCLS) {
         int cnt = 0;
@@ -529,6 +554,66 @@
         *ovf_count = 0;
         *pass_count = 0ull;
     }
+}
+
+__global__ __launch_bounds__(256) void k_scan(int32_t *__restrict__ blockhist, int nblocks,
+                                              MpbTables *__restrict__ tb, int nb, int32_t *__restrict__ ovf_count,
+                                              unsigned long long *__restrict__ pass_count, uint32_t *__restrict__ ticket)
+{
+    __shared__ int s_part[256];
+    __shared__ int s_last;
+    const int c = blockIdx.x, tid = threadIdx.x;
+    const int seg = (nblocks + 255) / 256;
+    const int b0 = tid * seg, b1 = min(nblocks, b0 + seg);
+    int sum = 0;
+    int32_t *bh = blockhist + (int64_t)c * nblocks;
+    int b = b0;
+    for (; b + 8 <= b1; b += 8) {
+        int v[8];
+#pragma unroll
+        for (int j = 0; j < 8; j++) v[j] = bh[b + j];
+#pragma unroll
+        for (int j = 0; j < 8; j++) sum += v[j];
+    }
+    for (; b < b1; b++) sum += bh[b];
+    s_part[tid] = sum;
+    __syncthreads();
+    for (int off = 1; off < 256; off <<= 1) {
+        int v = (tid >= off) ? s_part[tid - off] : 0;
+        __syncthreads();
+        s_part[tid] += v;
+        __syncthreads();
+    }
+    int run = s_part[tid] - sum;
+    for (b = b0; b + 8 <= b1; b += 8) {
+        int v[8];
+#pragma unroll
+        for (int j = 0; j < 8; j++) v[j] = bh[b + j];
+#pragma unroll
+        for (int j = 0; j < 8; j++) { bh[b + j] = run; run += v[j]; }
+    }
+    for (; b < b1; b++) {
+        const int h = bh[b];
+        bh[b] = run;
+        run += h;
+    }
+    if (tid == 255) tb->kcount[c] = s_part[255];
+    if (!ticket) return;
+    if (tid == 255) {
+        __threadfence();
+        s_last = atomicAdd(ticket, 1u) == gridDim.x - 1;
+    }
+    __syncthreads();
+    if (!s_last) return;
+    __threadfence();
+    build_tables(tb, nb, ovf_count, pass_count);
+    if (tid == 0) *ticket = 0u;
+}
+
+__global__ __launch_bounds__(256) void k_tables(MpbTables *__restrict__ tb, int nb, int32_t *__restrict__ ovf_count,
+                                                unsigned long long *__restrict__ pass_count)
+{
+    build_tables(tb, nb, ovf_count, pass_count);
 }
 
 __global__ void k_tables_overflow(MpbTables *__restrict__ tb, const int32_t *__restrict__ ovf_count,
@@ -604,6 +689,92 @@
         for (int k = tid; k < nkeys; k += 256)
             s_base[k] += s_wcnt[0][k] + s_wcnt[1][k] + s_wcnt[2][k] + s_wcnt[3][k];
         __syncthreads();
+    }
+}
+
+template <bool RAGGED>
+__global__ __launch_bounds__(256) void k_scatter_ranked(const uint8_t *__restrict__ cls, const uint16_t *__restrict__ rank, int64_t n,
+                                                        const int32_t *__restrict__ len_arg, int max_len, int len_shift,
+                                                        const int32_t *__restrict__ blockhist,
+                                                        const MpbTables *__restrict__ tb,
+                                                        const int32_t *__restrict__ ns,
+                                                        int32_t *__restrict__ perm, uint16_t *__restrict__ perm_ns,
+                                                        const int32_t *__restrict__ list)
+{
+    constexpr int nb = RAGGED ? MPB_LEN_BINS : 1;
+    constexpr int nkeys = MPB_NCLS * nb;
+    constexpr int kpt = (nkeys + 255) / 256;
+    static_assert(nkeys <= 256 * kpt && kpt <= 2, "a thread scans its own keys");
+    __shared__ int s_base[nkeys];
+    __shared__ int s_lstart[nkeys];
+    __shared__ int s_wsum[4];
+    __shared__ int s_id[MPB_PRE_READS], s_dst[MPB_PRE_READS];
+    __shared__ uint16_t s_ns[MPB_PRE_READS];
+    const int32_t *__restrict__ len = RAGGED ? len_arg : nullptr;
+    const int tid = threadIdx.x, w = tid >> 6, lane = tid & 63;
+    const int nblk = gridDim.x, blk = blockIdx.x;
+    const int slots = tb->perm_base[MPB_NCLS];
+    int c_r[MPB_PRE_ROUNDS], ns_r[MPB_PRE_ROUNDS], rk_r[MPB_PRE_ROUNDS], len_r[MPB_PRE_ROUNDS], id_r[MPB_PRE_ROUNDS];
+#pragma unroll
+    for (int round = 0; round < MPB_PRE_ROUNDS; round++) {
+        const int64_t k = (int64_t)blk * MPB_PRE_READS + round * 256 + tid;
+        const int64_t i = (list && k < n) ? (int64_t)list[k] : k;
+        id_r[round] = (int)i;
+        c_r[round] = k < n ? (int)cls[i] : 0xff;
+        rk_r[round] = k < n ? (int)rank[i] : 0;
+        ns_r[round] = k < n ? ns[i] : 0;
+        len_r[round] = (len && k < n) ? len[i] : 0;
+    }
+    int cnt[kpt], mine = 0;
+#pragma unroll
+    for (int j = 0; j < kpt; j++) {
+        const int k = tid * kpt + j;
+        cnt[j] = 0;
+        if (k < nkeys) {
+            const int h = blockhist[(int64_t)k * nblk + blk];
+            const int next = blk + 1 < nblk ? blockhist[(int64_t)k * nblk + blk + 1] : tb->kcount[k];
+            s_base[k] = tb->key_base[k] + h;
+            cnt[j] = next - h;
+        }
+        mine += cnt[j];
+    }
+    int incl = mine;
+#pragma unroll
+    for (int off = 1; off < 64; off <<= 1) {
+        const int v = __shfl_up(incl, off);
+        if (lane >= off) incl += v;
+    }
+    if (lane == 63) s_wsum[w] = incl;
+    __syncthreads();
+    int before = incl - mine;
+    for (int ww = 0; ww < w; ww++) before += s_wsum[ww];
+    const int total = min(MPB_PRE_READS, s_wsum[0] + s_wsum[1] + s_wsum[2] + s_wsum[3]);
+#pragma unroll
+    for (int j = 0; j < kpt; j++) {
+        const int k = tid * kpt + j;
+        if (k < nkeys) s_lstart[k] = before;
+        before += cnt[j];
+    }
+    __syncthreads();
+#pragma unroll
+    for (int round = 0; round < MPB_PRE_ROUNDS; round++) {
+        const int c = c_r[round] & 0x7f;
+        if (c_r[round] == 0xff || c >= MPB_NCLS) continue;
+        const int kk = c * nb + (len ? min(MPB_LEN_BINS - 1, clamp_len(len_r[round], max_len) >> len_shift) : 0);
+        const int at = s_lstart[kk] + rk_r[round];
+        if ((unsigned)at < (unsigned)MPB_PRE_READS) {
+            s_id[at] = id_r[round];
+            s_ns[at] = (uint16_t)ns_r[round];
+            s_dst[at] = s_base[kk] + rk_r[round];
+        }
+    }
+    __syncthreads();
+    for (int j = tid; j < total; j += 256) {
+        const int pos = s_dst[j];
+        if ((unsigned)pos < (unsigned)slots) {
+            perm[pos] = s_id[j];
+            perm_ns[pos] = s_ns[j];
+        }
     }
 }
 
@@ -775,27 +946,29 @@
 #undef MPB_DP_AR
 
 
-template <int AR>
+template <int AR, bool OVF = false>
 __device__ __forceinline__ void dp_grid(const DpArgs &args, DpArgs &s_args, const double2 *__restrict__ lut_g,
-                                        MpbTables *__restrict__ tb, const int32_t *__restrict__ perm, int chunk_tiles)
+                                        MpbTables *__restrict__ tb, const int32_t *__restrict__ perm, int chunk_tiles,
+                                        int ovf_class = 0)
 {
     mpb_s_lut[threadIdx.x] = lut_g[threadIdx.x];
     if (threadIdx.x == 0) { s_args = args; mpb_s_cells = 0ull; }
     __syncthreads();
     const DpArgs *A = &s_args;
-    const int total = tb->total_tiles;
+    const int ovf_cnt = OVF ? *args.ovf_count : 0;
+    const int total = OVF ? (ovf_cnt + 64 / c_classes[ovf_class].G - 1) / (64 / c_classes[ovf_class].G) : tb->total_tiles;
     const int nchunks = (total + chunk_tiles - 1) / chunk_tiles;
     for (int chunk = blockIdx.x * 4 + (threadIdx.x >> 6); chunk < nchunks; chunk += gridDim.x * 4) {
         const int t0 = chunk * chunk_tiles;
         const int t1 = min(total, t0 + chunk_tiles);
-        for (int c = MPB_NCLS - 1; c >= 0; c--) {
-            const int cnt = tb->count[c];
+        for (int c = OVF ? ovf_class : MPB_NCLS - 1; c >= (OVF ? ovf_class : 0); c--) {
+            const int cnt = OVF ? ovf_cnt : tb->count[c];
             const int rpt = 64 / c_classes[c].G;
-            const int s = tb->tile_start[c];
+            const int s = OVF ? 0 : tb->tile_start[c];
             const int e = s + (cnt + rpt - 1) / rpt;
             const int lo = max(t0, s), hi = min(t1, e);
             if (lo >= hi) continue;
-            const int32_t *pc = perm + tb->perm_base[c];
+            const int32_t *pc = OVF ? perm : perm + tb->perm_base[c];
             switch (c) {
 #define MPB_CASE(ID, RR, GG) case ID:                                                                 \
                 if constexpr (AR == MPB_AR_ODDS) dp_tiles_odds<RR, GG>(A, pc, cnt, lo - s, hi - lo);                \
@@ -817,10 +990,12 @@
 __global__ __launch_bounds__(256, MPB_DP_WAVES_PER_EU) void k_dp(DpArgs args,
                                             const double2 *__restrict__ lut_g,
                                             MpbTables *__restrict__ tb,
-                                            const int32_t *__restrict__ perm, int chunk_tiles)
+                                            const int32_t *__restrict__ perm, int chunk_tiles,
+                                            int ovf_class, long long *__restrict__ ovf_total)
 {
     __shared__ DpArgs s_args;
-    dp_grid<FMA ? MPB_AR_FMA : MPB_AR_EXACT>(args, s_args, lut_g, tb, perm, chunk_tiles);
+    if (OVERFLOW_PASS && blockIdx.x == 0 && threadIdx.x == 0) *ovf_total += *args.ovf_count;
+    dp_grid<FMA ? MPB_AR_FMA : MPB_AR_EXACT, OVERFLOW_PASS>(args, s_args, lut_g, tb, perm, chunk_tiles, ovf_class);
 }
 
 __global__ __launch_bounds__(256, MPB_DP_WAVES_PER_EU) void k_dp_odds(DpArgs args,
@@ -2080,7 +2255,7 @@
 {
 #define MPB_PRE_LAUNCH(RG, LG, LS)                                                                                      \
     hipLaunchKernelGGL((k_prepass<RG, LG, LS>), dim3(pre_blocks(n)), dim3(256), 0, s, q, n, stride, len, prm, o, ws.blockhist, list)
-    const PreOut o = {ws.cls, ns_out, ee_out, pass_out, ws.bad_len, ws.wide_list, ws.wide_rows, ws.wide_count};
+    const PreOut o = {ws.cls, ns_out, ee_out, pass_out, ws.bad_len, ws.wide_list, ws.wide_rows, ws.wide_count, ws.rank};
     const bool long_rows = prm.max_len > 16 * 12 * MPB_PRE_NB;
     if (list) {
         if (len) { if (long_rows) MPB_PRE_LAUNCH(true, true, true); else MPB_PRE_LAUNCH(true, false, true); }
@@ -2096,7 +2271,7 @@
                                 int64_t n, int64_t stride, const int32_t *len, const MpbDevParams &prm,
                                 const MpbWorkspace &ws, int32_t *ns_out, double *ee_out, uint8_t *pass_out, hipStream_t s)
 {
-    const PreOut o = {ws.cls, ns_out, ee_out, pass_out, ws.bad_len, ws.wide_list, ws.wide_rows, ws.wide_count};
+    const PreOut o = {ws.cls, ns_out, ee_out, pass_out, ws.bad_len, ws.wide_list, ws.wide_rows, ws.wide_count, ws.rank};
     const PreDecode dec = {seq, qual, out, offset, err};
     const uint8_t *q = out;
     const uint32_t cpr = (uint32_t)(stride >> 4);
@@ -2114,13 +2289,24 @@
 void mpb_launch_scan(int64_t n, const int32_t *len, const MpbWorkspace &ws, hipStream_t s)
 {
     const int nb = len ? MPB_LEN_BINS : 1;
-    hipLaunchKernelGGL(k_scan, dim3(MPB_NCLS * nb), dim3(256), 0, s, ws.blockhist, pre_blocks(n), ws.tables);
-    hipLaunchKernelGGL(k_tables, dim3(1), dim3(512), 0, s, ws.tables, nb, ws.ovf_count, ws.pass_count);
+    uint32_t *ticket = len ? nullptr : ws.scan_ticket;
+    hipLaunchKernelGGL(k_scan, dim3(MPB_NCLS * nb), dim3(256), 0, s, ws.blockhist, pre_blocks(n), ws.tables, nb, ws.ovf_count,
+                       ws.pass_count, ticket);
+    if (!ticket) hipLaunchKernelGGL(k_tables, dim3(1), dim3(256), 0, s, ws.tables, nb, ws.ovf_count, ws.pass_count);
 }
 
 void mpb_launch_scatter(int64_t n, const int32_t *len, const int32_t *ns, const MpbDevParams &prm, const MpbWorkspace &ws,
-                        hipStream_t s, const int32_t *list)
-{
+                        hipStream_t s, const int32_t *list, bool ranked)
+{
+    if (ranked) {
+        if (len)
+            hipLaunchKernelGGL((k_scatter_ranked<true>), dim3(pre_blocks(n)), dim3(256), 0, s, ws.cls, ws.rank, n, len, prm.max_len,
+                               prm.len_shift, ws.blockhist, ws.tables, ns, ws.perm, ws.perm_ns, list);
+        else
+            hipLaunchKernelGGL((k_scatter_ranked<false>), dim3(pre_blocks(n)), dim3(256), 0, s, ws.cls, ws.rank, n, len, prm.max_len,
+                               prm.len_shift, ws.blockhist, ws.tables, ns, ws.perm, ws.perm_ns, list);
+        return;
+    }
     if (len)
         hipLaunchKernelGGL((k_scatter<true>), dim3(pre_blocks(n)), dim3(256), 0, s, ws.cls, n, len, prm.max_len, prm.len_shift,
                            ws.blockhist, ws.tables, ns, ws.perm, ws.perm_ns, list);
@@ -2155,9 +2341,9 @@
     if (lut_odds)
         hipLaunchKernelGGL(k_dp_odds, dim3(blocks), dim3(256), 0, s, A, lut_odds, ws.tables, ws.perm, chunk_tiles);
     else if (prm.flags & MPB_FLAG_FAST_FMA)
-        hipLaunchKernelGGL((k_dp<true, false>), dim3(blocks), dim3(256), 0, s, A, ws.lut, ws.tables, ws.perm, chunk_tiles);
+        hipLaunchKernelGGL((k_dp<true, false>), dim3(blocks), dim3(256), 0, s, A, ws.lut, ws.tables, ws.perm, chunk_tiles, 0, (long long *)nullptr);
     else
-        hipLaunchKernelGGL((k_dp<false, false>), dim3(blocks), dim3(256), 0, s, A, ws.lut, ws.tables, ws.perm, chunk_tiles);
+        hipLaunchKernelGGL((k_dp<false, false>), dim3(blocks), dim3(256), 0, s, A, ws.lut, ws.tables, ws.perm, chunk_tiles, 0, (long long *)nullptr);
 }
 
 #define MPB_WIDE_GRID 1024
@@ -2196,10 +2382,9 @@
     int wc = MPB_NCLS - 1;
     for (int c = MPB_NCLS - 1; c >= 0; c--)
         if (classes[c].cap >= prm.max_len + 1) wc = c;
-    hipLaunchKernelGGL(k_tables_overflow, dim3(1), dim3(64), 0, s, ws.tables2, ws.ovf_count, wc, ws.ovf_total);
     DpArgs A = make_args(q, stride, len, prm, ws, ns, ee, pass, 1);
     const int blocks = 256;
-    hipLaunchKernelGGL((k_dp<false, true>), dim3(blocks), dim3(256), 0, s, A, ws.lut, ws.tables2, ws.ovf_list, MPB_DP_CHUNK);
+    hipLaunchKernelGGL((k_dp<false, true>), dim3(blocks), dim3(256), 0, s, A, ws.lut, ws.tables2, ws.ovf_list, MPB_DP_CHUNK, wc, ws.ovf_total);
 }
 
 void mpb_launch_lambda(const uint8_t *q, int64_t n, int64_t stride, const int32_t *len, int32_t fixed_len,
diff --git a/moira_amd/csrc/mpb_resident.cpp b/moira_amd/csrc/mpb_resident.cpp
--- a/moira_amd/csrc/mpb_resident.cpp
+++ b/moira_amd/csrc/mpb_resident.cpp
@@ -80,12 +80,12 @@
 
 static int filter_device_tail(mpb_ctx *c, const uint8_t *d_q, int64_t n, int64_t row_stride, const int32_t *d_len,
                               const MpbDevParams &prm, double *d_ee, int32_t *d_ns, uint8_t *d_pass, mpb_filter_counts *counts,
-                              const int32_t *d_list = nullptr)
+                              bool ranked, const int32_t *d_list = nullptr)
 {
     hipStream_t s = c->stream;
     const int32_t max_len = prm.max_len;
     { Span t(c, MPB_K_SCAN);     mpb_launch_scan(n, d_len, c->ws, s); }
-    { Span t(c, MPB_K_SCATTER);  mpb_launch_scatter(n, d_len, d_ns, prm, c->ws, s, d_list); }
+    { Span t(c, MPB_K_SCATTER);  mpb_launch_scatter(n, d_len, d_ns, prm, c->ws, s, d_list, ranked); }
     const double2 *lut_odds = (prm.flags & MPB_FLAG_ODDS) && c->ws.lut == c->d_lut ? c->d_lut_odds : nullptr;
     { Span t(c, MPB_K_DP);       mpb_launch_dp(d_q, n, row_stride, d_len, prm, c->ws, d_ns, d_ee, d_pass, s, lut_odds); }
     if (max_len + 1 > MPB_TILE_MAX_ROWS) { Span t(c, MPB_K_WIDE); mpb_launch_wide(d_q, row_stride, d_len, prm, c->ws, d_ns, d_ee, d_pass, s); }
@@ -112,7 +112,7 @@
     const MpbDevParams prm = make_dev_params(params, fixed_len, max_len);
     if (params->flags & MPB_FLAG_COUNT_CELLS) HIPCHK(hipMemsetAsync(c->ws.alg_cells, 0, sizeof(unsigned long long), c->stream));
     { Span t(c, MPB_K_PREPASS);  mpb_launch_prepass(d_q, n, row_stride, d_len, prm, c->ws, d_ns, d_ee, d_pass, c->stream, d_list); }
-    return filter_device_tail(c, d_q, n, row_stride, d_len, prm, d_ee, d_ns, d_pass, counts, d_list);
+    return filter_device_tail(c, d_q, n, row_stride, d_len, prm, d_ee, d_ns, d_pass, counts, true, d_list);
 }
 
 static int narrow_choose(mpb_ctx *c, const uint8_t *d_q, int64_t n, int64_t row_stride, const int32_t *d_len, int32_t fixed_len,
@@ -302,7 +302,7 @@
     c->classified.valid = false;
     c->classes_whole = true;
     const MpbDevParams prm = make_dev_params(params, fixed_len, max_len);
-    return filter_device_tail(c, d_q, n, row_stride, d_len, prm, d_ee, d_ns, d_pass, counts);
+    return filter_device_tail(c, d_q, n, row_stride, d_len, prm, d_ee, d_ns, d_pass, counts, false);
 }
 
 int mpb_encode_ascii_device(mpb_ctx *c, const uint8_t *d_q, int64_t n, int64_t row_stride, int32_t fastq_offset,
```
